# cita-cloud/consensus_overlord

Hardware: AMD Instinct MI355X
Metric: BLS12-381 vote verifications/sec (batch 4096) at 1/2/4/8 MI355X vs host blst (higher is better)
Workload: dtype u32; 1 GPU; config3: 4096 distinct-message precommit votes per GPU, RLC batch verify; batch_per_gpu=4096, global_batch=4096, parallelism=single GPU

## Files before the change

### consensus_overlord_amd/csrc/fpvm.hpp

```cpp
#pragma once
#include "bls/fp.hpp"

#if defined(__HIPCC__)
#define VM_FN __device__ __forceinline__
#else
#define VM_FN inline
struct uint4 {
  uint32_t x, y, z, w;
};
inline uint4 make_uint4(uint32_t a, uint32_t b, uint32_t c, uint32_t d) { return uint4{a, b, c, d}; }
#endif

namespace ovh {
namespace vm {

enum : uint32_t {
  OP_NOP = 0, OP_MULS = 1, OP_SGN0 = 2, OP_LEX = 3, OP_INV = 4, OP_LIN = 5, OP_SEL = 6, OP_EQ = 7,
  OP_AND = 8, OP_OR = 9, OP_XOR = 10, OP_ST = 11, OP_SELB = 12,
};

constexpr uint32_t PREFETCH = 6;

struct Out {
  uint32_t* base;
  uint32_t cap;
  uint32_t unit;
};
constexpr uint32_t CONST_BASE = 0x800;
constexpr uint32_t KZERO = 1, KTAB = 2;

VM_FN void ld_slot(Fp& r, const uint32_t* __restrict__ slots, const uint32_t* __restrict__ cst,
                   uint32_t ref) {
  const uint32_t* src = ((ref & CONST_BASE) ? cst : slots) + (ref & (CONST_BASE - 1)) * 12;
  const uint4* s4 = reinterpret_cast<const uint4*>(src);
  const uint4 a = s4[0], b = s4[1], c = s4[2];
  r.v[0] = a.x; r.v[1] = a.y; r.v[2] = a.z; r.v[3] = a.w;
  r.v[4] = b.x; r.v[5] = b.y; r.v[6] = b.z; r.v[7] = b.w;
  r.v[8] = c.x; r.v[9] = c.y; r.v[10] = c.z; r.v[11] = c.w;
}

VM_FN const uint4* slot_ptr(const uint32_t* __restrict__ slots, const uint32_t* __restrict__ cst, uint32_t ref) {
  return reinterpret_cast<const uint4*>(((ref & CONST_BASE) ? cst : slots) + (ref & (CONST_BASE - 1)) * 12);
}

#if defined(__HIPCC__)
typedef uint32_t u32x4 __attribute__((ext_vector_type(4)));
typedef const __attribute__((address_space(3))) uint32_t* lds_cptr;
VM_FN uint32_t lds_addr(const uint32_t* __restrict__ slots, const uint32_t* __restrict__ cst, uint32_t ref) {
  return (uint32_t)(uintptr_t)(lds_cptr)(((ref & CONST_BASE) ? cst : slots) + (ref & (CONST_BASE - 1)) * 12);
}
VM_FN void unpack4(Fp& r, int q, const u32x4 v) {
  r.v[4 * q] = v.x; r.v[4 * q + 1] = v.y; r.v[4 * q + 2] = v.z; r.v[4 * q + 3] = v.w;
}
#endif

VM_FN void ld_slots4(Fp& A, Fp& B, Fp& C, Fp& D, const uint32_t* __restrict__ slots,
                     const uint32_t* __restrict__ cst, uint32_t ra, uint32_t rb, uint32_t rc, uint32_t rd) {
#if defined(__HIPCC__) && defined(OVH_VM_ASM_LOADS)
  const uint32_t xa = lds_addr(slots, cst, ra), xb = lds_addr(slots, cst, rb), xc = lds_addr(slots, cst, rc),
                 xd = lds_addr(slots, cst, rd);
  u32x4 b0, d0, a0, c0, b1, d1, a1, c1, b2, d2, a2, c2;
  asm volatile(
      "ds_read_b128 %0, %12\n\tds_read_b128 %1, %13\n\tds_read_b128 %2, %14\n\tds_read_b128 %3, %15\n\t"
      "ds_read_b128 %4, %12 offset:16\n\tds_read_b128 %5, %13 offset:16\n\t"
      "ds_read_b128 %6, %14 offset:16\n\tds_read_b128 %7, %15 offset:16\n\t"
      "ds_read_b128 %8, %12 offset:32\n\tds_read_b128 %9, %13 offset:32\n\t"
      "ds_read_b128 %10, %14 offset:32\n\tds_read_b128 %11, %15 offset:32"
      : "=&v"(b0), "=&v"(d0), "=&v"(a0), "=&v"(c0), "=&v"(b1), "=&v"(d1), "=&v"(a1), "=&v"(c1), "=&v"(b2),
        "=&v"(d2), "=&v"(a2), "=&v"(c2)
      : "v"(xb), "v"(xd), "v"(xa), "v"(xc)
      : "memory");
  asm volatile("s_waitcnt lgkmcnt(8)" : "+v"(b0), "+v"(d0), "+v"(a0), "+v"(c0));
  unpack4(B, 0, b0); unpack4(D, 0, d0); unpack4(A, 0, a0); unpack4(C, 0, c0);
  asm volatile("s_waitcnt lgkmcnt(4)" : "+v"(b1), "+v"(d1), "+v"(a1), "+v"(c1));
  unpack4(B, 1, b1); unpack4(D, 1, d1); unpack4(A, 1, a1); unpack4(C, 1, c1);
  asm volatile("s_waitcnt lgkmcnt(0)" : "+v"(b2), "+v"(d2), "+v"(a2), "+v"(c2));
  unpack4(B, 2, b2); unpack4(D, 2, d2); unpack4(A, 2, a2); unpack4(C, 2, c2);
  return;
#endif
#if defined(__HIP_DEVICE_COMPILE__)
  typedef const __attribute__((address_space(3))) u32x4* lds_q;
  const uint32_t sb = (uint32_t)(uintptr_t)(lds_cptr)slots, cb = (uint32_t)(uintptr_t)(lds_cptr)cst;
  auto addr = [&](uint32_t ref) -> lds_q {
    const uint32_t m = (uint32_t)__builtin_amdgcn_sbfe((int32_t)ref, 11, 1);
    uint32_t base;
    asm("v_bfi_b32 %0, %1, %2, %3" : "=v"(base) : "v"(m), "v"(cb), "v"(sb));
    return (lds_q)(uintptr_t)(__builtin_amdgcn_ubfe(ref, 0, 11) * 48u + base);
  };
  const lds_q pa = addr(ra), pb = addr(rb), pc = addr(rc), pd = addr(rd);
#else
  const uint4 *pa = slot_ptr(slots, cst, ra), *pb = slot_ptr(slots, cst, rb), *pc = slot_ptr(slots, cst, rc),
              *pd = slot_ptr(slots, cst, rd);
#endif
#pragma unroll
  for (int q = 0; q < 3; ++q) {
#if defined(__HIP_DEVICE_COMPILE__)
    const u32x4 b = pb[q], d = pd[q], a = pa[q], c = pc[q];
#else
    const uint4 b = pb[q], d = pd[q], a = pa[q], c = pc[q];
#endif
    B.v[4 * q] = b.x; B.v[4 * q + 1] = b.y; B.v[4 * q + 2] = b.z; B.v[4 * q + 3] = b.w;
    D.v[4 * q] = d.x; D.v[4 * q + 1] = d.y; D.v[4 * q + 2] = d.z; D.v[4 * q + 3] = d.w;
    A.v[4 * q] = a.x; A.v[4 * q + 1] = a.y; A.v[4 * q + 2] = a.z; A.v[4 * q + 3] = a.w;
    C.v[4 * q] = c.x; C.v[4 * q + 1] = c.y; C.v[4 * q + 2] = c.z; C.v[4 * q + 3] = c.w;
#if defined(__HIPCC__)
    __builtin_amdgcn_sched_barrier(0);
#endif
  }
}

VM_FN void st_slot(uint32_t* __restrict__ slots, uint32_t dst, const Fp& z) {
  uint4* d4 = reinterpret_cast<uint4*>(slots + dst * 12);
  d4[0] = make_uint4(z.v[0], z.v[1], z.v[2], z.v[3]);
  d4[1] = make_uint4(z.v[4], z.v[5], z.v[6], z.v[7]);
  d4[2] = make_uint4(z.v[8], z.v[9], z.v[10], z.v[11]);
}

VM_FN void set_flag(Fp& z, uint32_t f) {
  fp_zero(z);
  z.v[0] = f;
}

constexpr uint32_t P2_LIMBS[12] = {
    P_LIMBS[0] << 1, (P_LIMBS[1] << 1) | (P_LIMBS[0] >> 31), (P_LIMBS[2] << 1) | (P_LIMBS[1] >> 31),
    (P_LIMBS[3] << 1) | (P_LIMBS[2] >> 31), (P_LIMBS[4] << 1) | (P_LIMBS[3] >> 31),
    (P_LIMBS[5] << 1) | (P_LIMBS[4] >> 31), (P_LIMBS[6] << 1) | (P_LIMBS[5] >> 31),
    (P_LIMBS[7] << 1) | (P_LIMBS[6] >> 31), (P_LIMBS[8] << 1) | (P_LIMBS[7] >> 31),
    (P_LIMBS[9] << 1) | (P_LIMBS[8] >> 31), (P_LIMBS[10] << 1) | (P_LIMBS[9] >> 31),
    (P_LIMBS[11] << 1) | (P_LIMBS[10] >> 31)};

VM_FN void canon(Fp& r, const Fp& a) {
  uint32_t d[12], br = 0;
#pragma unroll
  for (int j = 0; j < 12; ++j) d[j] = subc32(a.v[j], P_LIMBS[j], br, &br);
#pragma unroll
  for (int j = 0; j < 12; ++j) r.v[j] = br ? a.v[j] : d[j];
}

constexpr uint32_t NP_LIMBS[12] = {
    0u - P_LIMBS[0], ~P_LIMBS[1], ~P_LIMBS[2], ~P_LIMBS[3], ~P_LIMBS[4], ~P_LIMBS[5],
    ~P_LIMBS[6], ~P_LIMBS[7], ~P_LIMBS[8], ~P_LIMBS[9], ~P_LIMBS[10], ~P_LIMBS[11]};
static_assert(P_LIMBS[0] != 0, "NP_LIMBS: no borrow out of limb 0");

VM_FN uint32_t quot_est(uint32_t t) {
  constexpr float QS = (float)((1.0 - 0x1p-20) / (double)((P_LIMBS[11] >> 7) + 1));
  return (uint32_t)((float)t * QS);
}

VM_FN void scale_reduce(Fp& r, const uint32_t* s, uint32_t k) {
  const uint32_t q = quot_est(k * (uint32_t)((((uint64_t)s[12] << 32) | s[11]) >> 7));
  uint64_t acc = 0;
#pragma unroll
  for (int j = 0; j < 12; ++j) {
    acc = (uint64_t)k * s[j] + (acc >> 32);
    acc = (uint64_t)q * NP_LIMBS[j] + acc;
    r.v[j] = (uint32_t)acc;
  }
}

constexpr uint32_t P2P1_LIMBS[12] = {
    P2_LIMBS[0] + 1, P2_LIMBS[1], P2_LIMBS[2], P2_LIMBS[3], P2_LIMBS[4], P2_LIMBS[5],
    P2_LIMBS[6], P2_LIMBS[7], P2_LIMBS[8], P2_LIMBS[9], P2_LIMBS[10], P2_LIMBS[11]};

VM_FN void lin_mad(Fp& r, const Fp& A, const Fp& B, const Fp& C, const Fp& D, int ca, int cb, int cc, int cd) {
  const Fp* X[4] = {&A, &B, &C, &D};
  const int cf[4] = {ca, cb, cc, cd};
  uint64_t acc[12];
#pragma unroll
  for (int j = 0; j < 12; ++j) acc[j] = 0;
  uint32_t nw = 0;
#pragma unroll
  for (int t = 0; t < 4; ++t) {
    const uint32_t a = cf[t] < 0 ? (uint32_t)(-cf[t]) : (uint32_t)cf[t];
    const uint32_t m = cf[t] < 0 ? ~0u : 0u;
    nw += a & m;
#pragma unroll
    for (int j = 0; j < 12; ++j) acc[j] = (uint64_t)a * (X[t]->v[j] ^ m) + acc[j];
  }
#pragma unroll
  for (int j = 0; j < 12; ++j) acc[j] = (uint64_t)nw * P2P1_LIMBS[j] + acc[j];
  const int64_t top = (int64_t)(acc[11] >> 7) - ((int64_t)nw << 25);
  const uint32_t q = top > 0 ? quot_est((uint32_t)top) : 0u;
  uint64_t cy = 0;
#pragma unroll
  for (int j = 0; j < 12; ++j) {
    const uint64_t v = (uint64_t)q * NP_LIMBS[j] + (acc[j] + cy);
    r.v[j] = (uint32_t)v;
    cy = v >> 32;
  }
}

VM_FN void pre_add2(Fp& x, const Fp& A, const Fp& B, Fp& y, const Fp& C, const Fp& D, bool ny, bool any_neg) {
  uint32_t c1 = 0, c2 = 0;
  if (any_neg) {
    uint32_t nd[12], b2 = 0;
#pragma unroll
    for (int j = 0; j < 13; ++j) {
      if (j < 12) {
        nd[j] = subc32(P2_LIMBS[j], D.v[j], b2, &b2);
        x.v[j] = addc32(A.v[j], B.v[j], c1, &c1);
      }
      if (j >= 1) y.v[j - 1] = addc32(C.v[j - 1], ny ? nd[j - 1] : D.v[j - 1], c2, &c2);
    }
  } else {
#pragma unroll
    for (int j = 0; j < 12; ++j) {
      x.v[j] = addc32(A.v[j], B.v[j], c1, &c1);
      y.v[j] = addc32(C.v[j], D.v[j], c2, &c2);
    }
  }
}

constexpr uint32_t H_MUL = 1u << 22, H_MULNEG = 1u << 23, H_FLAG = 1u << 24, H_LIN = 1u << 25,
                   H_LINNEG = 1u << 26, H_ACC = 1u << 27, H_RARE = 1u << 28, H_SELB = 1u << 29,
                   H_LINNEG2 = 1u << 30, H_LINNEG3 = 1u << 31;
constexpr uint32_t H_ANY = H_MUL | H_LIN | H_ACC | H_RARE;

template <bool XB, bool XC>
VM_FN void lin_chain_neg(uint32_t* s, const Fp& A, const Fp& B, const Fp& C, const Fp& D, uint32_t mb, uint32_t mc,
                         uint32_t md, const Fp& K) {
  uint32_t u[12], v[12], w[12], c1 = 0, c2 = 0, c3 = 0, c4 = 0;
#pragma unroll
  for (int j = 0; j < 14; ++j) {
    if (j < 12) {
      u[j] = addc32(A.v[j], XB ? B.v[j] ^ mb : B.v[j], c1, &c1);
      v[j] = addc32(XC ? C.v[j] ^ mc : C.v[j], D.v[j] ^ md, c2, &c2);
    }
    if (j >= 1 && j <= 12) w[j - 1] = addc32(u[j - 1], v[j - 1], c3, &c3);
    if (j >= 2) s[j - 2] = addc32(w[j - 2], K.v[j - 2], c4, &c4);
  }
}

VM_FN void lin_sum(uint32_t* s, const Fp& A, const Fp& B, const Fp& C, const Fp& D, uint32_t mb, uint32_t mc,
                   uint32_t md, uint32_t hdr, const uint32_t* __restrict__ cst) {
  if (hdr & H_LINNEG) {
    const uint32_t n = (mb & 1u) + (mc & 1u) + (md & 1u);
    Fp K;
    ld_slot(K, nullptr, cst, CONST_BASE + KTAB + n);
    if (hdr & H_LINNEG3) {
      lin_chain_neg<true, true>(s, A, B, C, D, mb, mc, md, K);
    } else if (hdr & H_LINNEG2) {
#if defined(__HIP_DEVICE_COMPILE__)
      __asm__ volatile("");
#endif
      lin_chain_neg<false, true>(s, A, B, C, D, mb, mc, md, K);
    } else {
#if defined(__HIP_DEVICE_COMPILE__)
      __asm__ volatile("");
#endif
      lin_chain_neg<false, false>(s, A, B, C, D, mb, mc, md, K);
    }
  } else {
    uint32_t u[12], v[12], c1 = 0, c2 = 0, c3 = 0;
#pragma unroll
    for (int j = 0; j < 13; ++j) {
      if (j < 12) {
        u[j] = addc32(A.v[j], B.v[j], c1, &c1);
        v[j] = addc32(C.v[j], D.v[j], c2, &c2);
      }
      if (j >= 1) s[j - 1] = addc32(u[j - 1], v[j - 1], c3, &c3);
    }
  }
  s[12] = 0;
}

VM_FN void fp_inv(Fp& r, const Fp& a, const Fp& r3) { fp_inv_divsteps(r, a, r3); }

#if defined(__HIPCC__)
VM_FN uint32_t uniform(uint32_t w0) { return __builtin_amdgcn_readfirstlane(w0); }
#else
inline uint32_t uniform(uint32_t w0) { return w0; }
#endif

VM_FN uint32_t sign_mask(uint32_t w, int bit) { return (uint32_t)((int32_t)(w << (31 - bit)) >> 31); }
VM_FN int coef5(uint32_t w, int lo) { return ((int)(w << (27 - lo))) >> 27; }

VM_FN void exec(const uint4 in, bool active, uint32_t* __restrict__ slots, const uint32_t* __restrict__ cst,
                uint64_t scalar, const Out& out) {
  const uint32_t hdr = uniform(in.x);
  if (!(hdr & H_ANY)) return;
  const uint32_t op = active ? (in.x & 31) : (uint32_t)OP_NOP;
  uint32_t ra = in.y & 0xFFFF, rb = in.y >> 16, rc = in.z & 0xFFFF;
  bool selb = false;
  if (hdr & H_SELB) {
#if defined(__HIP_DEVICE_COMPILE__)
    __asm__ volatile("");
#endif
    selb = op == OP_SELB;
    const bool bit = ((scalar >> ((in.x >> 16) & 63)) & 1) != 0;
    ra = selb ? (bit ? rc : rb) : ra;
    rb = selb ? CONST_BASE + KZERO : rb;
    rc = selb ? CONST_BASE + KZERO : rc;
  }
  Fp A, B, C, D;
  ld_slots4(A, B, C, D, slots, cst, ra, rb, rc, in.z >> 16);
  const uint32_t dst = (in.x >> 5) & 0x7FF;
  const bool force_acc = (in.w & (1u << 24)) != 0;
  if (hdr & H_MUL) {
    const bool is_mul = op == OP_MULS || op == OP_SGN0 || op == OP_LEX || op == OP_EQ;
    Fp x, y, m;
    pre_add2(x, A, B, y, C, D, sign_mask(in.w, 19) != 0, (hdr & H_MULNEG) != 0);
    fp_mul(m, x, y);
    if (hdr & H_FLAG) {
      const bool flag = is_mul && op != OP_MULS;
      uint32_t f = 0;
      if (op == OP_SGN0) f = m.v[0] & 1u;
      if (op == OP_LEX) f = limbs_gt(m.v, HALF_P) ? 1u : 0u;
      if (op == OP_EQ) f = fp_is_zero(m) ? 1u : 0u;
#pragma unroll
      for (int j = 0; j < 12; ++j) m.v[j] = flag ? (j == 0 ? f : 0u) : m.v[j];
    }
    if (is_mul) st_slot(slots, dst, m);
  }
  if (hdr & H_LIN) {
    uint32_t s[13];
    lin_sum(s, A, B, C, D, sign_mask(in.w, 9), sign_mask(in.w, 14), sign_mask(in.w, 19), hdr, cst);
    const uint32_t k = (in.w >> 20) & 15;
    Fp l;
    scale_reduce(l, s, k > 1 ? k : 1u);
    if ((op == OP_LIN && !force_acc) || selb) st_slot(slots, dst, l);
  }
  if (hdr & H_ACC) {
    Fp l;
    lin_mad(l, A, B, C, D, coef5(in.w, 0), coef5(in.w, 5), coef5(in.w, 10), coef5(in.w, 15));
    if (op == OP_LIN && force_acc) st_slot(slots, dst, l);
  }
  if (hdr & H_RARE) {
    const bool rare = op != OP_NOP && op != OP_LIN && !selb && op != OP_MULS && op != OP_SGN0 && op != OP_LEX &&
                      op != OP_EQ;
    const uint32_t imm = (in.x >> 16) & 63;
    Fp z = A;
    if (op == OP_ST) {
      canon(z, A);
      uint32_t* b = out.base + (size_t)imm * 12 * out.cap + out.unit;
#pragma unroll
      for (int k = 0; k < 12; ++k) b[(size_t)k * out.cap] = z.v[k];
    } else if (op == OP_SEL) {
      z = A.v[0] ? C : B;
    } else if (op >= OP_AND && op <= OP_XOR) {
      set_flag(z, op == OP_AND ? (A.v[0] & C.v[0]) : op == OP_OR ? (A.v[0] | C.v[0]) : (A.v[0] ^ C.v[0]));
    } else if (op == OP_INV) {
#ifndef OVH_VM_NO_INV
      Fp a;
      canon(a, A);
      fp_inv(z, a, C);
#endif
    }
    if (rare && op != OP_ST) st_slot(slots, dst, z);
  }
#if defined(__HIP_DEVICE_COMPILE__)
  __asm__ volatile("" ::"v"(A.v[11]), "v"(B.v[11]), "v"(C.v[11]), "v"(D.v[11]));
#endif
}

#if defined(__HIPCC__)
constexpr uint32_t SIDE_VALID = 1u << 31, SIDE_FILL = 1u << 30;

__device__ __forceinline__ void side_spill(uint32_t sw, uint32_t* __restrict__ slots, uint32_t* __restrict__ scr) {
  if ((sw & (SIDE_VALID | SIDE_FILL)) == SIDE_VALID) {
    const u32x4* s = reinterpret_cast<const u32x4*>(slots + (sw & 0x7FF) * 12);
    const u32x4 a = s[0], b = s[1], c = s[2];
    u32x4* d = reinterpret_cast<u32x4*>(scr + ((sw >> 11) & 0xFFF) * 12);
    d[0] = a;
    d[1] = b;
    d[2] = c;
  }
}

template <bool SIDE = false>
__device__ __forceinline__ void run(const uint4* __restrict__ code, uint32_t nphases, uint32_t W, uint32_t lane,
                                    bool active, uint32_t* __restrict__ slots, const uint32_t* __restrict__ cst,
                                    uint64_t scalar, const Out& out, uint64_t* __restrict__ trace = nullptr,
                                    const uint32_t* __restrict__ side = nullptr, uint32_t* __restrict__ scr = nullptr) {
  static_assert(PREFETCH >= 5, "the unrolled loops below read up to 4 phases past the end");
  if constexpr (SIDE) {
    uint4 qa = code[lane], qb = code[W + lane], qc;
    uint32_t sa = side[lane], sb = side[W + lane], sc;
    if (!active) sa = sb = 0;
    __builtin_amdgcn_s_waitcnt(0x0F70);
    auto step = [&](const uint4& q, uint4& q2, const uint32_t s, const uint32_t sn, uint32_t& s2,
                    const uint32_t ph) __attribute__((always_inline)) {
      const bool fill = (sn & (SIDE_VALID | SIDE_FILL)) == (SIDE_VALID | SIDE_FILL);
      u32x4 f0, f1, f2;
      if (fill) {
        const u32x4* src = reinterpret_cast<const u32x4*>(scr + ((sn >> 11) & 0xFFF) * 12);
        f0 = __builtin_nontemporal_load(src);
        f1 = __builtin_nontemporal_load(src + 1);
        f2 = __builtin_nontemporal_load(src + 2);
      }
      q2 = code[(size_t)(ph + 2) * W + lane];
      s2 = active ? side[(size_t)(ph + 2) * W + lane] : 0u;
      exec(q, active, slots, cst, scalar, out);
      side_spill(s, slots, scr);
      if (fill) {
        u32x4* d = reinterpret_cast<u32x4*>(slots + (sn & 0x7FF) * 12);
        d[0] = f0;
        d[1] = f1;
        d[2] = f2;
      }
    };
#pragma unroll 1
    for (uint32_t ph = 0; ph < nphases; ph += 3) {
      step(qa, qc, sa, sb, sc, ph);
      step(qb, qa, sb, sc, sa, ph + 1);
      step(qc, qb, sc, sa, sb, ph + 2);
    }
    __asm__ volatile("s_waitcnt lgkmcnt(0)\n\ts_barrier" ::: "memory");
    return;
  }
  if (trace && threadIdx.x == 0) trace[0] = wall_clock64();
  uint4 qa = code[lane], qb = code[W + lane], qc;
  __builtin_amdgcn_s_waitcnt(0x0F70);
  auto step = [&](const uint4& q, uint4& q2, const uint32_t ph) __attribute__((always_inline)) {
    q2 = code[(size_t)(ph + 2) * W + lane];
    exec(q, active, slots, cst, scalar, out);
    if (trace && ph < nphases) {
      __asm__ volatile("s_waitcnt lgkmcnt(0)" ::: "memory");
      if (threadIdx.x == 0) trace[ph + 1] = wall_clock64();
    }
  };
#pragma unroll 1
  for (uint32_t ph = 0; ph < nphases; ph += 3) {
    step(qa, qc, ph);
    step(qb, qa, ph + 1);
    step(qc, qb, ph + 2);
  }
  __asm__ volatile("s_waitcnt lgkmcnt(0)\n\ts_barrier" ::: "memory");
}

#endif

}
}
```

### consensus_overlord_amd/csrc/msm.hpp

```cpp
#pragma once

#define MSM_NBW 255
#define MSM_NB (4 * MSM_NBW)
#define MSM_NT 32
#define MSM_TM 64
#define MSM_LV 27
#define MSM_U (MSM_NT * MSM_TM)
#define MSM_CH_LV 6
#define MSM_CH (1u << MSM_CH_LV)
#define MSM_PF_ROWS 2

struct MsmArgs {
  const uint32_t* cnt;
  const uint32_t* off;
  const uint32_t* pf;
  const uint32_t* ent;
  Slab st;
  Slab A;
  Slab U;
};

__device__ __forceinline__ uint32_t msm_half(uint64_t r, uint32_t h) { return h ? (uint32_t)(r >> 32) : (uint32_t)r; }

#define MSM_TPB 64

__global__ __launch_bounds__(MSM_TPB) void k_msm_zero(uint32_t* __restrict__ cnt) {
  const uint32_t k = blockIdx.x * MSM_TPB + threadIdx.x;
  if (k < MSM_NB) cnt[k] = 0;
}

__global__ __launch_bounds__(MSM_TPB) void k_msm_count(uint32_t n, uint64_t seed, uint64_t base,
                                                       const int32_t* __restrict__ codes, uint32_t* __restrict__ cnt) {
  __shared__ uint32_t h[MSM_NB];
  for (uint32_t k = threadIdx.x; k < MSM_NB; k += MSM_TPB) h[k] = 0;
  __syncthreads();
  const uint32_t i = blockIdx.x * MSM_TPB + threadIdx.x;
  if (i < n && codes[i] == 0) {
    const uint64_t r = vote_scalar(seed, base, i);
    for (uint32_t hh = 0; hh < 2; ++hh) {
      const uint32_t s = msm_half(r, hh);
      for (uint32_t w = 0; w < 4; ++w) {
        const uint32_t d = (s >> (8 * w)) & 255u;
        if (d) atomicAdd(&h[w * MSM_NBW + d - 1], 1u);
      }
    }
  }
  __syncthreads();
  for (uint32_t k = threadIdx.x; k < MSM_NB; k += MSM_TPB)
    if (h[k]) atomicAdd(&cnt[k], h[k]);
}

template <class F, class G>
__device__ __forceinline__ uint32_t wave_scan_nb(F v, G out) {
  static_assert(MSM_NB <= 16 * 64, "16 entries per lane");
  const uint32_t t = threadIdx.x;
  uint32_t loc[16], sum = 0;
#pragma unroll
  for (int j = 0; j < 16; ++j) {
    const uint32_t b = 16 * t + j;
    loc[j] = b < MSM_NB ? v(b) : 0u;
    sum += loc[j];
  }
  uint32_t incl = sum;
#pragma unroll
  for (int d = 1; d < 64; d <<= 1) {
    const uint32_t x = __shfl_up(incl, d, 64);
    if (t >= (uint32_t)d) incl += x;
  }
  uint32_t run = incl - sum;
#pragma unroll
  for (int j = 0; j < 16; ++j) {
    const uint32_t b = 16 * t + j;
    if (b < MSM_NB) out(b, run);
    run += loc[j];
  }
  return __shfl(incl, 63, 64);
}

__global__ __launch_bounds__(64) void k_msm_scan(const uint32_t* __restrict__ cnt, uint32_t* __restrict__ off,
                                                 uint32_t* __restrict__ cur, uint32_t* __restrict__ pf) {
  const uint32_t tot = wave_scan_nb([&](uint32_t b) { return cnt[b]; },
                                    [&](uint32_t b, uint32_t e) {
                                      off[b] = e;
                                      cur[b] = e;
                                    });
  if (threadIdx.x == 0) off[MSM_NB] = tot;
  for (uint32_t row = 0; row < MSM_PF_ROWS; ++row) {
    uint32_t* p = pf + (size_t)row * (MSM_NB + 1);
    const uint32_t t = wave_scan_nb(
        [&](uint32_t b) {
          const uint32_t c = cnt[b];
          return row == 0 ? (c + 1) / 2 : (c + MSM_CH - 1) >> MSM_CH_LV;
        },
        [&](uint32_t b, uint32_t e) { p[b] = e; });
    if (threadIdx.x == 0) p[MSM_NB] = t;
  }
}

__global__ __launch_bounds__(MSM_TPB) void k_msm_scatter(uint32_t n, uint64_t seed, uint64_t base,
                                                         const int32_t* __restrict__ codes, uint32_t* __restrict__ cur,
                                                         uint32_t* __restrict__ ent) {
  const uint32_t i = blockIdx.x * MSM_TPB + threadIdx.x;
  if (i >= n || codes[i] != 0) return;
  const uint64_t r = vote_scalar(seed, base, i);
  for (uint32_t hh = 0; hh < 2; ++hh) {
    const uint32_t s = msm_half(r, hh);
    for (uint32_t w = 0; w < 4; ++w) {
      const uint32_t d = (s >> (8 * w)) & 255u;
      if (d) ent[atomicAdd(&cur[w * MSM_NBW + d - 1], 1u)] = 2 * i + hh;
    }
  }
}

__global__ __launch_bounds__(64) void k_sig_as_S(Slab st, const int32_t* __restrict__ codes, Slab U) {
  const uint32_t c = threadIdx.x;
  if (c >= 6) return;
  Fp v;
  const bool ok = codes[0] == 0;
  if (ok && c < 4) st.ld(v, S_SIG + c, 0);
  else if (c == (ok ? 4u : 2u)) fp_one(v);
  else fp_zero(v);
  U.st(v, c, 0);
}

enum : uint32_t { SRC_ID = 0, SRC_PT = 1, SRC_A = 2, SRC_U = 3 };

__device__ __forceinline__ uint32_t msm_find(const uint32_t* __restrict__ row, uint32_t q) {
  uint32_t lo = 0, hi = MSM_NB;
  while (hi - lo > 1) {
    const uint32_t mid = (lo + hi) >> 1;
    if (row[mid] <= q) lo = mid;
    else hi = mid;
  }
  return lo;
}

__device__ __forceinline__ uint32_t msm_member(uint32_t j, uint32_t k) {
  return ((j >> k) << (k + 1)) | (1u << k) | (j & ((1u << k) - 1));
}

__device__ __forceinline__ void msm_coord(Fp& v, const MsmArgs& a, uint32_t kind, uint32_t idx, uint32_t c) {
  if (kind == SRC_PT) {
    if (c < 4) a.st.ld(v, ((idx & 1) ? S_TAU : S_SIG) + c, idx >> 1);
    else if (c == 4) fp_one(v);
    else fp_zero(v);
  } else if (kind == SRC_A) {
    a.A.ld(v, c, idx);
  } else if (kind == SRC_U) {
    a.U.ld(v, c, idx);
  } else if (c == 2) {
    fp_one(v);
  } else {
    fp_zero(v);
  }
}

template <int W>
__device__ __forceinline__ void msm_pair_op(const VmDev& prog, uint32_t nin, uint32_t* slots, const uint32_t* cst,
                                            uint32_t lane, bool active, const MsmArgs& a, uint32_t ka, uint32_t ia,
                                            uint32_t kb, uint32_t ib, uint32_t kd, uint32_t id) {
  if (active) {
    const uint32_t na = nin - 6;
    for (uint32_t k = lane; k < nin; k += W) {
      Fp v;
      if (k < na) msm_coord(v, a, ka, ia, k);
      else msm_coord(v, a, kb, ib, k - na);
      slot_put(slots, prog.in[k], v.v);
    }
  }
  __syncthreads();
  vm::run(prog.code, prog.nphases, W, lane, active, slots, cst, 0, vm::Out{nullptr, 0, 0});
  if (active) {
    const Slab& d = kd == SRC_U ? a.U : a.A;
    for (uint32_t k = lane; k < 6; k += W) {
      Fp v;
      const uint32_t src = prog.out[k];
      for (int l = 0; l < 12; ++l) v.v[l] = slots[src * 12 + l];
      vm::canon(v, v);
      d.st(v, k, id);
    }
  }
  __syncthreads();
}

__device__ __forceinline__ VmDev msm_prog(bool first, const VmDev& x, const VmDev& y) {
  VmDev r;
  r.code = first ? x.code : y.code;
  r.nphases = first ? x.nphases : y.nphases;
  r.in = first ? x.in : y.in;
  r.out = first ? x.out : y.out;
  r.trace = nullptr, r.clk = nullptr, r.side = nullptr;
  return r;
}

#define MSM_VM_PROLOGUE(W)                                    \
  __builtin_amdgcn_s_setprio(3);                              \
  extern __shared__ uint4 lds4[];                             \
  uint32_t* lds = reinterpret_cast<uint32_t*>(lds4);          \
  const uint32_t* cst = lds;                                  \
  const uint32_t slice = threadIdx.x / (W), lane = threadIdx.x % (W); \
  uint32_t* slots = lds + SLOT_BASE_W + slice * stride_w;     \
  load_consts(lds, cst_g, VM_NCONST)

__global__ __launch_bounds__(64) void k_msm_chunk(VmDev madd, VmDev padd, uint32_t stride_w,
                                                  const uint32_t* __restrict__ cst_g, MsmArgs a) {
  constexpr uint32_t W = VM_MADD_W, SL = 64 / W;
  const uint32_t* rowc = a.pf + (MSM_NB + 1);
  if (blockIdx.x >= rowc[MSM_NB]) return;
  MSM_VM_PROLOGUE(W);
  const uint32_t b = msm_find(rowc, blockIdx.x), k0 = (blockIdx.x - rowc[b]) << MSM_CH_LV;
  const uint32_t c = a.cnt[b], a0 = a.pf[b], e0 = a.off[b];
  const uint32_t m = c - k0 < MSM_CH ? c - k0 : MSM_CH;
  for (uint32_t lv = 0; lv < MSM_CH_LV && (lv == 0 || (1u << lv) < m); ++lv) {
    const uint32_t h = 1u << lv;
    const uint32_t np = lv == 0 ? (m + 1) / 2 : (m - h + 2 * h - 1) >> (lv + 1);
    const VmDev prog = msm_prog(lv == 0, madd, padd);
    for (uint32_t r = 0; r < np; r += SL) {
      const uint32_t p = r + slice, k = k0 + (p << (lv + 1));
      const bool act = p < np;
      uint32_t ka = SRC_A, ia = a0 + (k >> 1), kb = SRC_A, ib = a0 + ((k + h) >> 1);
      const uint32_t id = ia;
      if (lv == 0) {
        ka = SRC_PT, kb = SRC_ID, ia = ib = 0;
        if (act) {
          ia = a.ent[e0 + k];
          if (k + 1 < c) kb = SRC_PT, ib = a.ent[e0 + k + 1];
        }
      }
      msm_pair_op<W>(prog, lv == 0 ? VM_MADD_NIN : VM_PADD_NIN, slots, cst, lane, act, a, ka, ia, kb, ib, SRC_A, id);
    }
  }
}

__global__ __launch_bounds__(64) void k_msm_upper(VmDev padd, uint32_t stride_w, const uint32_t* __restrict__ cst_g,
                                                  MsmArgs a) {
  constexpr uint32_t W = VM_PADD_W, SL = 64 / W;
  const uint32_t c = a.cnt[blockIdx.x];
  if (c <= MSM_CH) return;
  MSM_VM_PROLOGUE(W);
  const uint32_t a0 = a.pf[blockIdx.x];
  for (uint32_t lv = MSM_CH_LV; (1u << lv) < c; ++lv) {
    const uint32_t h = 1u << lv, np = (c - h + 2 * h - 1) >> (lv + 1);
    for (uint32_t r = 0; r < np; r += SL) {
      const uint32_t p = r + slice, k = p << (lv + 1);
      const uint32_t ia = a0 + (k >> 1), ib = a0 + ((k + h) >> 1);
      msm_pair_op<W>(padd, VM_PADD_NIN, slots, cst, lane, p < np, a, SRC_A, ia, SRC_A, ib, SRC_A, ia);
    }
  }
}

__global__ __launch_bounds__(64) void k_msm_plane(uint32_t lo, uint32_t hi, VmDev padd, uint32_t stride_w,
                                                  const uint32_t* __restrict__ cst_g, MsmArgs a) {
  constexpr uint32_t W = VM_PADD_W, SL = 64 / W;
  MSM_VM_PROLOGUE(W);
  const uint32_t per_t = MSM_TM >> hi, t = blockIdx.x / per_t, g = blockIdx.x % per_t;
  for (uint32_t lv = lo; lv <= hi; ++lv) {
    const uint32_t np = 1u << (hi - lv);
    for (uint32_t r = 0; r < np; r += SL) {
      const uint32_t p = r + slice, i = g * np + p;
      const bool act = p < np;
      uint32_t ka = SRC_U, ia = t * MSM_TM + (i << lv), kb = SRC_U, ib = ia + (lv ? 1u << (lv - 1) : 0u);
      const uint32_t id = ia;
      if (lv == 0) {
        ka = kb = SRC_ID, ia = ib = 0;
        if (act) {
          const uint32_t w = t >> 3, k = t & 7;
          const uint32_t b0 = w * MSM_NBW + msm_member(2 * i, k) - 1, b1 = w * MSM_NBW + msm_member(2 * i + 1, k) - 1;
          if (a.cnt[b0]) ka = SRC_A, ia = a.pf[b0];
          if (a.cnt[b1]) kb = SRC_A, ib = a.pf[b1];
        }
      }
      msm_pair_op<W>(padd, VM_PADD_NIN, slots, cst, lane, act, a, ka, ia, kb, ib, SRC_U, id);
    }
  }
}

__global__ __launch_bounds__(64) void k_msm_comb(uint32_t lo, uint32_t hi, VmDev p0, VmDev p1, VmDev p2,
                                                 uint32_t stride_w, const uint32_t* __restrict__ cst_g, MsmArgs a) {
  constexpr uint32_t W = VM_HDBL1_W, SL = 64 / W;
  MSM_VM_PROLOGUE(W);
  for (uint32_t h = lo; h <= hi; ++h) {
    const VmDev prog = msm_prog(h == lo, p0, msm_prog(h == lo + 1, p1, p2));
    const uint32_t np = 1u << (hi - h), m = 1u << (h - 1);
    for (uint32_t r = 0; r < np; r += SL) {
      const uint32_t p = r + slice, e = 2 * m * (blockIdx.x * np + p) * MSM_TM;
      msm_pair_op<W>(prog, VM_HDBL1_NIN, slots, cst, lane, p < np, a, SRC_U, e, SRC_U, e + m * MSM_TM, SRC_U, e);
    }
  }
}
```

### consensus_overlord_amd/csrc/ovhip.hip

```cpp
#include <hip/hip_runtime.h>

#include <errno.h>
#include <stdlib.h>
#include <sys/random.h>
#include <sys/types.h>

#include <algorithm>
#include <atomic>
#include <deque>
#include <mutex>
#include <new>
#include <string>
#include <string.h>
#include <unordered_map>
#include <vector>

#include "../../include/ovhip.h"
#include "bls/verify.hpp"
#include "fpvm.hpp"
#include "keygen.hpp"
#include "rlp.hpp"
#include "sm3.hpp"
#ifdef OVH_VM_PROGS
#include OVH_VM_PROGS
#else
#include <vm_progs.inc>
#endif
static_assert(VM_KZERO == ovh::vm::KZERO && VM_KTAB == ovh::vm::KTAB, "fixed constants (tools/fpvm/gen.py)");

using namespace ovh;

#define WG 64

struct Slab {
  uint32_t* p;
  uint32_t cap;
  __device__ __forceinline__ void ld(Fp& a, uint32_t j, uint32_t i) const {
    const uint32_t* b = p + (size_t)j * 12 * cap + i;
#pragma unroll
    for (int k = 0; k < 12; ++k) a.v[k] = b[(size_t)k * cap];
  }
  __device__ __forceinline__ void st(const Fp& a, uint32_t j, uint32_t i) const {
    uint32_t* b = p + (size_t)j * 12 * cap + i;
#pragma unroll
    for (int k = 0; k < 12; ++k) b[(size_t)k * cap] = a.v[k];
  }
  __device__ void ld2(Fp2& a, uint32_t j, uint32_t i) const {
    ld(a.c0, j, i);
    ld(a.c1, j + 1, i);
  }
  __device__ void st2(const Fp2& a, uint32_t j, uint32_t i) const {
    st(a.c0, j, i);
    st(a.c1, j + 1, i);
  }
  __device__ void ld_g2j(G2J& a, uint32_t i) const {
    ld2(a.X, 0, i);
    ld2(a.Y, 2, i);
    ld2(a.Z, 4, i);
  }
  __device__ void st_g2j(const G2J& a, uint32_t i) const {
    st2(a.X, 0, i);
    st2(a.Y, 2, i);
    st2(a.Z, 4, i);
  }
  __device__ void ld_g2a(G2A& a, uint32_t i) const {
    ld2(a.x, 0, i);
    ld2(a.y, 2, i);
  }
  __device__ void st_g2a(const G2A& a, uint32_t i) const {
    st2(a.x, 0, i);
    st2(a.y, 2, i);
  }
  __device__ void ld_g1a(G1A& a, uint32_t i) const {
    ld(a.x, 0, i);
    ld(a.y, 1, i);
  }
  __device__ void st_g1a(const G1A& a, uint32_t i) const {
    st(a.x, 0, i);
    st(a.y, 1, i);
  }
  __device__ void ld_f12(Fp12& f, uint32_t i) const {
    Fp* c = &f.c0.c0.c0;
    for (int j = 0; j < 12; ++j) ld(c[j], j, i);
  }
  __device__ void st_f12(const Fp12& f, uint32_t i) const {
    const Fp* c = &f.c0.c0.c0;
    for (int j = 0; j < 12; ++j) st(c[j], j, i);
  }
};

enum : uint32_t {
  S_U = VM_S_U,
  S_SIG = VM_S_SIG,
  S_TAU = VM_S_TAU,
  S_F = VM_S_F,
  S_RS = VM_S_RS,
  S_TOTAL = VM_S_TOTAL,
};
constexpr uint32_t PART_PLANES = 18;
constexpr size_t FIN_STRIDE = (size_t)PART_PLANES * 12 * 20;

enum : int { ST_H2F = 0, ST_VOTE, ST_FOLD, ST_FINAL, ST_FALLBACK, ST_MSM };
static_assert(ST_MSM + 1 == OVH_NSTAGES, "stage table");

__device__ __forceinline__ uint64_t rlc_scalar(uint64_t seed, uint64_t i) {
  uint64_t z = seed + 0x9e3779b97f4a7c15ull * (i + 1);
  z = (z ^ (z >> 30)) * 0xbf58476d1ce4e5b9ull;
  z = (z ^ (z >> 27)) * 0x94d049bb133111ebull;
  z = z ^ (z >> 31);
  return z ? z : 1;
}

#define UNIT_BASE 0xFFFFFFFFFFFFFFFFull
__device__ __forceinline__ uint64_t vote_scalar(uint64_t seed, uint64_t base, uint64_t i) {
  return base == UNIT_BASE ? 1ull : rlc_scalar(seed, base + i);
}

__global__ __launch_bounds__(WG) void k_vote_digest(uint32_t n, const uint64_t* __restrict__ heights,
                                                    const uint64_t* __restrict__ rounds,
                                                    const uint8_t* __restrict__ types, const uint8_t* __restrict__ bh,
                                                    const uint8_t* __restrict__ lens, uint8_t* __restrict__ out) {
  const uint32_t i = blockIdx.x * WG + threadIdx.x;
  if (i >= n) return;
  uint8_t h[VOTE_HASH_MAX];
  const uint32_t len = lens[i];
  uint8_t d[32];
  if (len > VOTE_HASH_MAX) {
    for (int k = 0; k < 32; ++k) out[(size_t)i * 32 + k] = 0;
    return;
  }
  for (uint32_t k = 0; k < len; ++k) h[k] = bh[(size_t)i * VOTE_HASH_MAX + k];
  vote_digest(d, heights[i], rounds[i], types[i], h, len);
  for (int k = 0; k < 32; ++k) out[(size_t)i * 32 + k] = d[k];
}

__global__ __launch_bounds__(WG) void k_h2f(uint32_t n, const uint8_t* __restrict__ hashes, XmdTemplates t, Slab s) {
  const uint32_t i = blockIdx.x * WG + threadIdx.x;
  if (i >= n) return;
  uint32_t msg[8], uni[64];
  be_words_from_bytes(msg, hashes + (size_t)i * 32, 8);
  expand_message_xmd_256(uni, msg, t);
  Fp2 u0, u1;
  hash_to_field_fp2x2(u0, u1, uni);
  s.st2(u0, S_U, i);
  s.st2(u1, S_U + 2, i);
}

__device__ void parse_hdr(const uint8_t* b, uint32_t nbytes, uint32_t* x_hi, uint32_t* x_lo, uint32_t& bad,
                          uint32_t& inf, uint32_t& sort, uint32_t& xzero) {
  const uint8_t b0 = b[0];
  bad = 0;
  inf = 0;
  sort = (b0 >> 5) & 1u;
  xzero = 0;
  uint8_t t[48];
  for (int i = 0; i < 48; ++i) t[i] = b[i];
  t[0] &= 0x1f;
  limbs_from_be48(x_hi, t);
  if (nbytes == 96) limbs_from_be48(x_lo, b + 48);
  if (!(b0 & 0x80)) {
    bad = 1;
    return;
  }
  if (b0 & 0x40) {
    uint32_t acc = b0 & 0x3f;
    for (uint32_t i = 1; i < nbytes; ++i) acc |= b[i];
    if (acc) bad = 1;
    else inf = 1;
    return;
  }
  if (!limbs_lt_p(x_hi)) bad = 1;
  if (nbytes == 96 && !limbs_lt_p(x_lo)) bad = 1;
  uint32_t z = 0;
  for (int k = 0; k < 12; ++k) z |= x_hi[k] | (nbytes == 96 ? x_lo[k] : 0u);
  xzero = z == 0;
}

struct VmDev {
  const uint4* code;
  uint32_t nphases;
  const uint16_t* in;
  const uint16_t* out;
  uint64_t* trace;
  uint64_t* clk;
  const uint32_t* side;
};
constexpr uint32_t VOTE_NSCR = VM_VOTE_NSCR > VM_VOTE_T_NSCR ? VM_VOTE_NSCR : VM_VOTE_T_NSCR;

#define VM_CLOCK_WGS (1u << 16)
struct ClockStamp {
  uint64_t t0 = 0, r0 = 0;
  __device__ __forceinline__ void begin(const uint64_t* clk) {
    if (clk && threadIdx.x == 0) {
      t0 = __builtin_amdgcn_s_memtime();
      r0 = __builtin_amdgcn_s_memrealtime();
    }
  }
  __device__ __forceinline__ void end(uint64_t* clk) {
    if (clk && threadIdx.x == 0 && blockIdx.x < VM_CLOCK_WGS) {
      const uint64_t t1 = __builtin_amdgcn_s_memtime(), r1 = __builtin_amdgcn_s_memrealtime();
      clk[2 * blockIdx.x] = t1 - t0;
      clk[2 * blockIdx.x + 1] = r1 - r0;
    }
  }
};

#ifndef SMALL_MAX
#define SMALL_MAX 1024u
#endif
#define VM_SLICES 4
constexpr uint32_t align128w(uint32_t w) { return (w + 31) / 32 * 32; }
constexpr uint32_t align256w(uint32_t w) { return (w + 63) / 64 * 64; }
constexpr uint32_t SLOT_BASE_W = align256w(VM_NCONST * 12);
constexpr uint32_t VOTE_STRIDE_W = align256w(VM_VOTE_NSLOTS * 12 + 4);
constexpr uint32_t VOTE_T_STRIDE_W = align256w(VM_VOTE_T_NSLOTS * 12 + 4);
constexpr uint32_t FOLD_STRIDE_W = align128w(VM_FOLD_NSLOTS * 12);
#define VM_FOLD_UNITS (64 / VM_FOLD_W)

__device__ __forceinline__ void load_consts(uint32_t* cst, const uint32_t* __restrict__ g, uint32_t n) {
  for (uint32_t k = threadIdx.x; k < n * 12; k += blockDim.x) cst[k] = g[k];
}

__device__ __forceinline__ void slot_flag(uint32_t* slots, uint32_t s, uint32_t f) {
  uint4* d = reinterpret_cast<uint4*>(slots + s * 12);
  d[0] = make_uint4(f, 0, 0, 0);
  d[1] = make_uint4(0, 0, 0, 0);
  d[2] = make_uint4(0, 0, 0, 0);
}

__device__ __forceinline__ void slot_put(uint32_t* slots, uint32_t s, const uint32_t* v) {
  for (int k = 0; k < 12; ++k) slots[s * 12 + k] = v[k];
}

__device__ __forceinline__ uint32_t slot_flag_get(const uint32_t* slots, uint32_t s) { return slots[s * 12]; }

__device__ __forceinline__ void fold_unit(uint32_t t, uint32_t m, const VmDev& prog, const uint32_t* cst,
                                          uint32_t* slots, uint32_t lane, bool active, Slab inF, Slab inS,
                                          Slab out, const int32_t* __restrict__ codes) {
  if (active) {
    for (uint32_t k = lane; k < 4 * PART_PLANES; k += VM_FOLD_W) {
      const uint32_t q = k / PART_PLANES, j = k % PART_PLANES, e = 4 * t + q;
      Fp v;
      if (e < m && (!codes || codes[e] == 0) && (j < 12 || inS.p)) {
        if (j < 12) inF.ld(v, j, e);
        else inS.ld(v, j - 12, e);
      } else if (j == 0 || j == 12 + 2) {
        fp_one(v);
      } else {
        fp_zero(v);
      }
      slot_put(slots, VM_FOLD_IN[k], v.v);
    }
  }
  __syncthreads();
  vm::run(prog.code, VM_FOLD_NPHASES, VM_FOLD_W, lane, active, slots, cst, 0, vm::Out{nullptr, 0, 0});
  if (active) {
    for (uint32_t k = lane; k < PART_PLANES; k += VM_FOLD_W) {
      Fp v;
      const uint32_t src = VM_FOLD_OUT[k];
      for (int q = 0; q < 12; ++q) v.v[q] = slots[src * 12 + q];
      vm::canon(v, v);
      out.st(v, k, t);
    }
  }
}

#ifndef OVH_VOTE_STAGGER
#define OVH_VOTE_STAGGER 12
#endif
__device__ __forceinline__ void vote_stagger() {
#if OVH_VOTE_STAGGER > 0
  const uint32_t hw = __builtin_amdgcn_s_getreg((31 << 11) | 4);
  const uint32_t n = ((hw >> 4) & 3) * OVH_VOTE_STAGGER;
#pragma unroll 1
  for (uint32_t k = 0; k < n; ++k) __builtin_amdgcn_s_sleep(1);
#endif
}

#define PKF_PARSE 1u
#define PKF_INF 2u
#define PKF_GRP 4u
struct PkSrc {
  const uint32_t* planes;
  uint32_t cap;
  const uint32_t* flags;
  const int32_t* idx;
};

#define POOL_SEQR 16u
#define POOL_QW 16u
enum : uint32_t {
  PQ_CUR = 0,
  PQ_NPUB = POOL_QW,
  PQ_SLOTOF = 2 * POOL_QW,
  PQ_NANN = 3 * POOL_QW,
  PQ_DONE = 4 * POOL_QW,
  PQ_CLAIM = PQ_DONE + OVH_BATCH_SLOTS * POOL_QW,
  PQ_INFL = PQ_CLAIM + OVH_BATCH_SLOTS * POOL_QW,
  PQ_OCC = PQ_INFL + POOL_QW,
};
constexpr uint32_t POOL_OCC_N = 4096;
constexpr uint32_t PQ_WORDS = PQ_OCC + POOL_OCC_N / 2;
static_assert(POOL_SEQR > OVH_BATCH_SLOTS && POOL_SEQR / 2 <= POOL_QW, "pool queue layout");
#define POOL_IDLE_TICKS 2000ull
#define POOL_WAIT_TICKS 2000000ull

__device__ __forceinline__ uint32_t simd_key() {
  const uint32_t hw = __builtin_amdgcn_s_getreg((31 << 11) | 4);
  const uint32_t xcc = __builtin_amdgcn_s_getreg((3 << 11) | 20);
  return (xcc & 7u) << 9 | ((hw >> 13) & 3u) << 7 | ((hw >> 12) & 1u) << 6 | ((hw >> 8) & 15u) << 2 |
         ((hw >> 4) & 3u);
}
__device__ __forceinline__ uint32_t* pq_occ(uint64_t* q) { return reinterpret_cast<uint32_t*>(q + PQ_OCC); }
#define POOL_SPREAD_TICKS 20000ull

struct PoolBatch {
  uint64_t seq;
  uint32_t n, nq;
  uint32_t table;
  uint32_t has_idx;
  uint64_t seed, base;
  int32_t* codes;
  const uint32_t* planes;
  const uint32_t* flags;
  uint32_t pcap, cap;
  uint32_t* state;
  uint32_t* part0;
  const uint8_t* stage;
  uint64_t* clk;
  uint32_t part_cap, pad;
  uint64_t* plog;
};

#define PLOG_RING 64u
#define PLOG_QUADS 1024u
#define PLOG_WORDS (16u + 2u * PLOG_QUADS)
#define PLOG_GRIDS 64u
#define PLOG_WGS 1024u
#define PLOG_WG_WORDS 4u
#define PLOG_GRID_BASE ((size_t)PLOG_RING * PLOG_WORDS)
#define PLOG_TOTAL (PLOG_GRID_BASE + (size_t)PLOG_GRIDS * (4 + PLOG_WGS * PLOG_WG_WORDS))
enum : uint32_t { PLOG_EV_PUB = 0, PLOG_EV_DONE = 1, PLOG_EV_FOLD = 2, PLOG_EV_MSM = 3, PLOG_EV_FINAL = 4,
                  PLOG_EV_BACK = 5, PLOG_EV_GATH = 6, PLOG_EV_COMB = 7, PLOG_EV_FE = 8, PLOG_EV_SEQ = 15 };
__global__ void k_grid_hdr(uint64_t* g, uint64_t seq, uint32_t par, uint32_t wgs) {
  for (uint32_t k = threadIdx.x; k < PLOG_WGS * PLOG_WG_WORDS; k += blockDim.x) g[4 + k] = 0;
  __syncthreads();
  if (threadIdx.x == 0) {
    g[0] = seq;
    g[1] = par;
    g[2] = wgs;
    g[3] = __builtin_amdgcn_s_memrealtime();
  }
}
__global__ void k_stamp(uint64_t* p, uint64_t v) {
  if (threadIdx.x == 0) {
    p[0] = __builtin_amdgcn_s_memrealtime();
    if (v != ~0ull) p[PLOG_EV_SEQ] = v;
  }
}

struct PoolArgs {
  uint64_t* q;
  const PoolBatch* descs;
  const uint4* pv_code;
  const uint32_t* pv_side;
  const uint4* pt_code;
  const uint32_t* pt_side;
  const uint4* fold_code;
  const uint32_t* cst;
  uint32_t* scr;
  uint64_t* wlog;
  uint64_t only;
  uint32_t nsimd;
  uint32_t skip_cu;
};

__device__ __forceinline__ uint64_t* pq_done(uint64_t* q, uint32_t slot) { return q + PQ_DONE + slot * POOL_QW; }
__device__ __forceinline__ uint64_t* pq_claim(uint64_t* q, uint32_t slot) { return q + PQ_CLAIM + slot * POOL_QW; }
__device__ __forceinline__ uint32_t* pq_slot_of(uint64_t* q) { return reinterpret_cast<uint32_t*>(q + PQ_SLOTOF); }
__device__ __forceinline__ uint64_t qld(const uint64_t* p) {
  return __hip_atomic_load(p, __ATOMIC_RELAXED, __HIP_MEMORY_SCOPE_AGENT);
}

__global__ __launch_bounds__(64) void k_pool_publish(PoolBatch b, uint32_t slot, uint64_t seq, uint64_t* q,
                                                     PoolBatch* descs) {
  if (threadIdx.x) return;
  b.seq = ~0ull;
  descs[slot] = b;
  __builtin_amdgcn_fence(__ATOMIC_RELEASE, "agent");
  asm volatile("s_waitcnt vmcnt(0)" ::: "memory");
  __hip_atomic_store(&descs[slot].seq, seq, __ATOMIC_RELAXED, __HIP_MEMORY_SCOPE_AGENT);
  __hip_atomic_store(pq_done(q, slot), 0ull, __ATOMIC_RELAXED, __HIP_MEMORY_SCOPE_AGENT);
  __hip_atomic_store(pq_claim(q, slot), seq << 32, __ATOMIC_RELAXED, __HIP_MEMORY_SCOPE_AGENT);
  __hip_atomic_store(pq_slot_of(q) + seq % POOL_SEQR, slot, __ATOMIC_RELAXED, __HIP_MEMORY_SCOPE_AGENT);
  __builtin_amdgcn_fence(__ATOMIC_RELEASE, "agent");
  asm volatile("s_waitcnt vmcnt(0)" ::: "memory");
  __hip_atomic_store(q + PQ_NPUB, seq + 1, __ATOMIC_RELAXED, __HIP_MEMORY_SCOPE_AGENT);
}

__global__ __launch_bounds__(64) void k_pool_announce(uint64_t* q, uint64_t n) {
  if (threadIdx.x == 0) __hip_atomic_store(q + PQ_NANN, n, __ATOMIC_RELAXED, __HIP_MEMORY_SCOPE_AGENT);
}

__device__ __forceinline__ uint64_t lane0_fetch_add(uint64_t* p, uint64_t v) {
  uint64_t r = 0;
  if (threadIdx.x == 0) r = __hip_atomic_fetch_add(p, v, __ATOMIC_RELAXED, __HIP_MEMORY_SCOPE_AGENT);
  return ((uint64_t)__builtin_amdgcn_readfirstlane((uint32_t)(r >> 32)) << 32) |
         __builtin_amdgcn_readfirstlane((uint32_t)r);
}
__device__ __forceinline__ uint32_t lane0_fetch_add32(uint32_t* p, uint32_t v) {
  uint32_t r = 0;
  if (threadIdx.x == 0) r = __hip_atomic_fetch_add(p, v, __ATOMIC_RELAXED, __HIP_MEMORY_SCOPE_AGENT);
  return __builtin_amdgcn_readfirstlane(r);
}
__device__ __forceinline__ void lane0_cas(uint64_t* p, uint64_t expect, uint64_t want) {
  if (threadIdx.x == 0) {
    uint64_t e = expect;
    (void)__hip_atomic_compare_exchange_strong(p, &e, want, __ATOMIC_RELAXED, __ATOMIC_RELAXED,
                                               __HIP_MEMORY_SCOPE_AGENT);
  }
}
__device__ __forceinline__ uint64_t wclock() {
  const uint64_t t = wall_clock64();
  return ((uint64_t)__builtin_amdgcn_readfirstlane((uint32_t)(t >> 32)) << 32) | __builtin_amdgcn_readfirstlane((uint32_t)t);
}
__device__ __forceinline__ uint64_t qldu(const uint64_t* p) {
  const uint64_t v = __hip_atomic_load(p, __ATOMIC_RELAXED, __HIP_MEMORY_SCOPE_AGENT);
  return ((uint64_t)__builtin_amdgcn_readfirstlane((uint32_t)(v >> 32)) << 32) | __builtin_amdgcn_readfirstlane((uint32_t)v);
}
__device__ uint32_t pool_claim(uint64_t* q, const PoolBatch* descs, uint32_t* slot_out, uint32_t* quad_out,
                               uint32_t* why, uint64_t only, uint32_t nsimd, uint32_t* how) {
  uint64_t t0 = wclock(), tdef = 0;
  uint32_t hw = 0;
  uint32_t* occ = pq_occ(q) + simd_key();
  *why = 3;
#pragma unroll 1
  for (uint32_t tries = 0; tries < (1u << 22); ++tries) {
    const uint64_t s = qldu(q + PQ_CUR), np = qldu(q + PQ_NPUB);
    if (s > only) {
      *why = 4;
      return 0;
    }
    if (s >= np) {
      const uint64_t idle = wclock() - t0;
      if (idle > POOL_WAIT_TICKS ||
          (idle > POOL_IDLE_TICKS && qldu(q + PQ_NANN) <= np && qldu(q + PQ_INFL) == 0)) {
        *why = idle > POOL_WAIT_TICKS ? 2 : 1;
        return 0;
      }
      if (idle > POOL_IDLE_TICKS) __builtin_amdgcn_s_sleep(127);
      else __builtin_amdgcn_s_sleep(8);
      continue;
    }
    const uint32_t slot = __builtin_amdgcn_readfirstlane(
        __hip_atomic_load(pq_slot_of(q) + s % POOL_SEQR, __ATOMIC_RELAXED, __HIP_MEMORY_SCOPE_AGENT));
    bool held = false;
    if (np == s + 1) {
      hw |= 1u;
      bool busy;
      if (tdef && __builtin_amdgcn_readfirstlane(__hip_atomic_load(occ, __ATOMIC_RELAXED, __HIP_MEMORY_SCOPE_AGENT))) {
        busy = true;
      } else {
        busy = lane0_fetch_add32(occ, 1u) != 0;
        held = true;
      }
      if (busy) {
        hw |= 2u;
        const uint64_t cw = qldu(pq_claim(q, slot));
        const uint32_t nq = __builtin_amdgcn_readfirstlane(
            __hip_atomic_load(&descs[slot].nq, __ATOMIC_RELAXED, __HIP_MEMORY_SCOPE_AGENT));
        const uint64_t infl = qldu(q + PQ_INFL);
        const uint32_t taken = (uint32_t)cw;
        if ((cw >> 32) == s && taken < nq && (uint64_t)(nq - taken) + infl <= nsimd + nsimd / 16) {
          const uint64_t now = wclock();
          if (!tdef) tdef = now;
          if (now - tdef < POOL_SPREAD_TICKS) {
            hw |= 4u;
            if (held) (void)lane0_fetch_add32(occ, ~0u);
            __builtin_amdgcn_s_sleep(32);
            continue;
          }
        }
        hw |= 8u;
      }
    }
    if (!held) (void)lane0_fetch_add32(occ, 1u);
    const uint64_t old = lane0_fetch_add(pq_claim(q, slot), 1ull);
    const uint64_t seq = old >> 32;
    const uint32_t idx = (uint32_t)old;
    const uint64_t tw = wclock();
    while (qldu(q + PQ_NPUB) <= seq && wclock() - tw < 100000000ull) __builtin_amdgcn_s_sleep(2);
    const uint32_t nq = __builtin_amdgcn_readfirstlane(
        __hip_atomic_load(&descs[slot].nq, __ATOMIC_RELAXED, __HIP_MEMORY_SCOPE_AGENT));
    asm volatile("s_waitcnt vmcnt(0)" ::: "memory");
    const uint64_t dseq = qldu(&descs[slot].seq);
    const bool mine = dseq == seq && idx < nq;
    if (seq != s || !mine) lane0_cas(q + PQ_CUR, s, s + 1);
    if (mine) {
      (void)lane0_fetch_add(q + PQ_INFL, 1ull);
      *slot_out = slot;
      *quad_out = idx;
      *how = hw;
      return 1;
    }
    (void)lane0_fetch_add32(occ, ~0u);
    tdef = 0;
    t0 = wclock();
  }
  return 0;
}

template <typename T>
__device__ __forceinline__ T dget(const T* p) {
  return __hip_atomic_load(p, __ATOMIC_RELAXED, __HIP_MEMORY_SCOPE_AGENT);
}
template <typename T>
__device__ __forceinline__ T* dgetp(T* const* p) {
  return reinterpret_cast<T*>(__hip_atomic_load(reinterpret_cast<const uint64_t*>(p), __ATOMIC_RELAXED,
                                                __HIP_MEMORY_SCOPE_AGENT));
}
__device__ __forceinline__ uint32_t uni(uint32_t v) { return __builtin_amdgcn_readfirstlane(v); }
__device__ __forceinline__ uint64_t uni64(uint64_t v) {
  return ((uint64_t)uni((uint32_t)(v >> 32)) << 32) | uni((uint32_t)v);
}
template <typename T>
__device__ __forceinline__ T* unip(T* p) {
  return reinterpret_cast<T*>(uni64(reinterpret_cast<uint64_t>(p)));
}

template <bool TABLE>
__device__ __forceinline__ void vote_quad(const PoolArgs& a, uint32_t slot_in, uint32_t quad_in, uint32_t* lds) {
  constexpr uint32_t NSLOTS = TABLE ? VM_VOTE_T_NSLOTS : VM_VOTE_NSLOTS;
  constexpr uint32_t STRIDE = TABLE ? VOTE_T_STRIDE_W : VOTE_STRIDE_W;
  constexpr uint32_t NPH = TABLE ? VM_VOTE_T_NPHASES : VM_VOTE_NPHASES;
  const uint16_t* IN = TABLE ? VM_VOTE_T_IN : VM_VOTE_IN;
  const uint16_t* OUT = TABLE ? VM_VOTE_T_OUT : VM_VOTE_OUT;
  uint32_t* cst = lds;
  const uint32_t slice = threadIdx.x / VM_VOTE_W, lane = threadIdx.x % VM_VOTE_W;
  uint32_t* slots = lds + SLOT_BASE_W + slice * STRIDE;
  uint32_t* hdr = slots + NSLOTS * 12;
  uint32_t* park = lds + SLOT_BASE_W + 2 * STRIDE + NSLOTS * 12 + 2;
  {
    const PoolBatch* bd = a.descs + slot_in;
    const uint32_t i = (quad_in & 0x0FFFFFFFu) * VM_SLICES + slice;
    const uint32_t n = uni(dget(&bd->n));
    const bool active = i < n;
    const uint8_t* sigs = unip(dgetp(&bd->stage));
    const Slab s{unip(dgetp(&bd->state)), uni(dget(&bd->cap))};
    if (active) {
      if (lane == 0) {
        uint32_t x1[12], x0[12], bad, inf, sort, xz;
        parse_hdr(sigs + (size_t)i * 96, 96, x1, x0, bad, inf, sort, xz);
        slot_put(slots, IN[TABLE ? VM_VOTE_T_IN_SIG_X1 : VM_VOTE_IN_SIG_X1], x1);
        slot_put(slots, IN[TABLE ? VM_VOTE_T_IN_SIG_X0 : VM_VOTE_IN_SIG_X0], x0);
        slot_flag(slots, IN[TABLE ? VM_VOTE_T_IN_SIG_SORT : VM_VOTE_IN_SIG_SORT], sort);
        hdr[0] = bad | inf << 1 | xz << 2;
      } else if (lane >= 2 && lane < 6) {
        Fp u;
        s.ld(u, S_U + (lane - 2), i);
        slot_put(slots, IN[(TABLE ? VM_VOTE_T_IN_U00 : VM_VOTE_IN_U00) + (lane - 2)], u.v);
      }
    }
    if (threadIdx.x == 0) {
      park[0] = slot_in;
      park[1] = quad_in;
      if (dgetp(&bd->plog)) {
        uint32_t* h3 = lds + SLOT_BASE_W + 3 * STRIDE + NSLOTS * 12 + 2;
        const uint64_t t = __builtin_amdgcn_s_memrealtime();
        h3[0] = (uint32_t)t;
        h3[1] = (uint32_t)(t >> 32);
      }
    }
    __syncthreads();
    if (active) {
      if constexpr (TABLE) {
        const int32_t* idx = reinterpret_cast<const int32_t*>(sigs + (size_t)n * 144);
        const uint32_t e = uni(dget(&bd->has_idx)) ? (uint32_t)idx[i] : i;
        if (lane == 1) {
          hdr[1] = unip(dgetp(&bd->flags))[e];
        } else if (lane >= 6 && lane < 9) {
          Fp v;
          Slab{const_cast<uint32_t*>(unip(dgetp(&bd->planes))), uni(dget(&bd->pcap))}.ld(v, lane - 6, e);
          slot_put(slots, IN[VM_VOTE_T_IN_PK_X + (lane - 6)], v.v);
        }
      } else {
        if (lane == 1) {
          uint32_t x[12], bad, inf, sort, xz;
          parse_hdr(sigs + (size_t)n * 96 + (size_t)i * 48, 48, x, x, bad, inf, sort, xz);
          slot_put(slots, IN[VM_VOTE_IN_PK_X], x);
          slot_flag(slots, IN[VM_VOTE_IN_PK_SORT], sort);
          hdr[1] = bad | inf << 1 | xz << 2;
        }
      }
    }
    if (threadIdx.x == 0 && dgetp(&bd->clk)) {
      const uint64_t t0 = __builtin_amdgcn_s_memtime(), r0 = __builtin_amdgcn_s_memrealtime();
      uint32_t* h0 = lds + SLOT_BASE_W + NSLOTS * 12 + 2;
      uint32_t* h1 = lds + SLOT_BASE_W + STRIDE + NSLOTS * 12 + 2;
      h0[0] = (uint32_t)t0;
      h0[1] = (uint32_t)(t0 >> 32);
      h1[0] = (uint32_t)r0;
      h1[1] = (uint32_t)(r0 >> 32);
    }
    __syncthreads();
    const uint64_t scalar = vote_scalar(uni64(dget(&bd->seed)), uni64(dget(&bd->base)), i);
    vm::run<true>(TABLE ? a.pt_code : a.pv_code, NPH, VM_VOTE_W, lane, active, slots, cst, scalar,
                  vm::Out{s.p, s.cap, i}, nullptr, TABLE ? a.pt_side : a.pv_side,
                  a.scr + (size_t)blockIdx.x * VM_SLICES * VOTE_NSCR * 12 + slice * VOTE_NSCR * 12);
  }
  const uint32_t slot = uni(park[0]), quad = uni(park[1]) & 0x0FFFFFFFu, how = uni(park[1]) >> 28;
  const PoolBatch* bd = a.descs + slot;
  const uint32_t i = quad * VM_SLICES + slice;
  const uint32_t n = uni(dget(&bd->n));
  int32_t* codes = unip(dgetp(&bd->codes));
  if (uint64_t* clk = dgetp(&bd->clk); clk && threadIdx.x == 0 && blockIdx.x < VM_CLOCK_WGS) {
    const uint32_t* h0 = lds + SLOT_BASE_W + NSLOTS * 12 + 2;
    const uint32_t* h1 = lds + SLOT_BASE_W + STRIDE + NSLOTS * 12 + 2;
    const uint64_t t0 = h0[0] | (uint64_t)h0[1] << 32, r0 = h1[0] | (uint64_t)h1[1] << 32;
    clk[2 * blockIdx.x] = __builtin_amdgcn_s_memtime() - t0;
    clk[2 * blockIdx.x + 1] = __builtin_amdgcn_s_memrealtime() - r0;
  }
  if (i < n && lane == 0) {
    const uint32_t sf = hdr[0], pf = hdr[1];
    const uint32_t sg_bad = sf & 1, sg_inf = (sf >> 1) & 1, sg_xz = (sf >> 2) & 1;
    const uint32_t sg_ok = slot_flag_get(slots, OUT[TABLE ? VM_VOTE_T_OUT_SIG_OK : VM_VOTE_OUT_SIG_OK]);
    const uint32_t sg_grp = slot_flag_get(slots, OUT[TABLE ? VM_VOTE_T_OUT_SIG_GRP : VM_VOTE_OUT_SIG_GRP]);
    const uint32_t h_inf = slot_flag_get(slots, OUT[TABLE ? VM_VOTE_T_OUT_H_INF : VM_VOTE_OUT_H_INF]);
    uint32_t pk_parse, pk_inf, pk_grp;
    if constexpr (TABLE) {
      pk_parse = pf & PKF_PARSE;
      pk_inf = pf & PKF_INF;
      pk_grp = !(pf & PKF_GRP);
    } else {
      const uint32_t pk_bad = pf & 1, pk_xz = (pf >> 2) & 1;
      pk_inf = (pf >> 1) & 1;
      const uint32_t pk_ok = slot_flag_get(slots, OUT[VM_VOTE_OUT_PK_OK]);
      pk_grp = slot_flag_get(slots, OUT[VM_VOTE_OUT_PK_GRP]);
      pk_parse = pk_bad || (!pk_inf && (!pk_ok || pk_xz));
    }
    int32_t c;
    if (pk_parse) c = OVH_ERR_PUBKEY;
    else if (sg_bad) c = BLST_BAD_ENCODING;
    else if (!sg_inf && !sg_ok) c = BLST_POINT_NOT_ON_CURVE;
    else if (!sg_inf && (sg_xz || !sg_grp)) c = BLST_POINT_NOT_IN_GROUP;
    else if (pk_inf) c = BLST_PK_IS_INFINITY;
    else if (!pk_grp) c = BLST_POINT_NOT_IN_GROUP;
    else if (h_inf || sg_inf) c = BLST_VERIFY_FAIL;
    else c = 0;
    codes[i] = c;
  }
  __threadfence();
  __syncthreads();
  uint64_t* const pl = threadIdx.x == 0 && quad < PLOG_QUADS ? dgetp(&bd->plog) : nullptr;
  uint64_t pl_start = 0;
  if (pl) {
    const uint32_t* h3 = lds + SLOT_BASE_W + 3 * STRIDE + NSLOTS * 12 + 2;
    pl_start = (uint64_t)h3[0] | (uint64_t)(h3[1] & 0xFFFFu) << 32;
  }
  const Slab s{unip(dgetp(&bd->state)), uni(dget(&bd->cap))};
  VmDev fold{};
  fold.code = a.fold_code;
  fold_unit(quad, n, fold, cst, lds + SLOT_BASE_W, threadIdx.x % VM_FOLD_W, threadIdx.x < VM_FOLD_W,
            Slab{s.p + (size_t)S_F * 12 * s.cap, s.cap}, Slab{nullptr, 0},
            Slab{unip(dgetp(&bd->part0)), uni(dget(&bd->part_cap))}, codes);
  if (pl) {
    pl[16 + 2 * quad] = pl_start | (uint64_t)simd_key() << 48 | (uint64_t)how << 60;
    pl[16 + 2 * quad + 1] = __builtin_amdgcn_s_memrealtime();
  }
  __builtin_amdgcn_fence(__ATOMIC_RELEASE, "agent");
  asm volatile("s_waitcnt vmcnt(0)" ::: "memory");
  if (threadIdx.x == 0) {
    __hip_atomic_fetch_add(pq_done(a.q, slot), 1ull, __ATOMIC_RELAXED, __HIP_MEMORY_SCOPE_AGENT);
    __hip_atomic_fetch_add(a.q + PQ_INFL, ~0ull, __ATOMIC_RELAXED, __HIP_MEMORY_SCOPE_AGENT);
    __hip_atomic_fetch_add(pq_occ(a.q) + simd_key(), ~0u, __ATOMIC_RELAXED, __HIP_MEMORY_SCOPE_AGENT);
  }
}

__global__ __launch_bounds__(64, 2) void k_vm_pool(PoolArgs a) {
  __builtin_amdgcn_s_setprio(2);
  extern __shared__ uint4 lds4[];
  if (a.skip_cu && ((simd_key() >> 2) & 0x7Fu) < a.skip_cu) return;
  uint32_t* lds = reinterpret_cast<uint32_t*>(lds4);
  load_consts(lds, a.cst, VM_NCONST);
  const uint64_t t_in = __builtin_amdgcn_s_memrealtime();
  vote_stagger();
  uint32_t nquads = 0, why = 0;
#pragma unroll 1
  for (;; ++nquads) {
    uint32_t slot = 0, quad = 0, how = 0;
    if (!pool_claim(a.q, a.descs, &slot, &quad, &why, a.only, a.nsimd, &how)) break;
    slot = uni(slot);
    quad = uni(quad) | uni(how) << 28;
    __builtin_amdgcn_fence(__ATOMIC_ACQUIRE, "agent");
    if (uni(dget(&a.descs[slot].table))) vote_quad<true>(a, slot, quad, lds);
    else vote_quad<false>(a, slot, quad, lds);
  }
  if (a.wlog && threadIdx.x == 0 && blockIdx.x < PLOG_WGS) {
    uint64_t* w = a.wlog + (size_t)blockIdx.x * PLOG_WG_WORDS;
    w[0] = t_in;
    w[1] = __builtin_amdgcn_s_memrealtime();
    w[2] = nquads;
    w[3] = why;
  }
}

__global__ __launch_bounds__(64) void k_pool_wait(uint64_t* q, uint32_t slot, uint32_t nq, uint64_t ticks,
                                                  uint32_t* err) {
  if (threadIdx.x) return;
  const uint64_t t0 = wall_clock64();
  while (__hip_atomic_load(pq_done(q, slot), __ATOMIC_RELAXED, __HIP_MEMORY_SCOPE_AGENT) < nq) {
    if (wall_clock64() - t0 > ticks) {
      __hip_atomic_store(err, 1u, __ATOMIC_RELAXED, __HIP_MEMORY_SCOPE_SYSTEM);
      return;
    }
    __builtin_amdgcn_s_sleep(32);
  }
}

__global__ __launch_bounds__(WG) void k_pool_stage(uint32_t n, const uint8_t* __restrict__ sigs,
                                                   const uint8_t* __restrict__ pks, const int32_t* __restrict__ idx,
                                                   uint8_t* __restrict__ dst) {
  const size_t nb = (size_t)n * 96 + (pks ? (size_t)n * 48 : 0);
  uint8_t* di = dst + (size_t)n * 144;
  for (size_t k = (size_t)blockIdx.x * WG + threadIdx.x; k < nb + (idx ? (size_t)n * 4 : 0);
       k += (size_t)gridDim.x * WG) {
    if (k < (size_t)n * 96) dst[k] = sigs[k];
    else if (k < nb) dst[k] = pks[k - (size_t)n * 96];
    else di[k - nb] = reinterpret_cast<const uint8_t*>(idx)[k - nb];
  }
}

template <int SLICES>
__global__ __launch_bounds__(64) void k_vm_fold(uint32_t m, VmDev prog, const uint32_t* __restrict__ cst_g, Slab inF,
                                                Slab inS, Slab out, const int32_t* __restrict__ codes,
                                                const int32_t* __restrict__ gate = nullptr) {
  if (gate && *gate == 1) return;
  __builtin_amdgcn_s_setprio(2);
  extern __shared__ uint4 lds4[];
  uint32_t* lds = reinterpret_cast<uint32_t*>(lds4);
  uint32_t* cst = lds;
  const uint32_t slice = threadIdx.x / VM_FOLD_W, lane = threadIdx.x % VM_FOLD_W;
  const uint32_t sl = slice < SLICES ? slice : 0;
  uint32_t* slots = lds + SLOT_BASE_W + sl * FOLD_STRIDE_W;
  const uint32_t t = blockIdx.x * SLICES + slice;
  const bool active = slice < SLICES && 4 * t < m;
  load_consts(cst, cst_g, VM_NCONST);
  fold_unit(t, m, prog, cst, slots, lane, active, inF, inS, out, codes);
}

__global__ __launch_bounds__(64) void k_vm_final(uint32_t m, VmDev prog, const uint32_t* __restrict__ cst_g, Slab inF,
                                                 Slab inS, Slab xS, int32_t* __restrict__ result) {
  __builtin_amdgcn_s_setprio(3);
  extern __shared__ uint4 lds4[];
  uint32_t* lds = reinterpret_cast<uint32_t*>(lds4);
  uint32_t* cst = lds;
  uint32_t* slots = lds + SLOT_BASE_W;
  const uint32_t lane = threadIdx.x;
  load_consts(cst, cst_g, VM_NCONST);
  for (uint32_t k = lane; k < 4 * PART_PLANES; k += 64) {
    const uint32_t q = k / PART_PLANES, j = k % PART_PLANES;
    Fp v;
    if (q == 0 && j >= 12 && xS.p) {
      xS.ld(v, j - 12, 0);
    } else if (q < m) {
      if (j < 12) inF.ld(v, j, q);
      else inS.ld(v, j - 12, q);
    } else if (j == 0 || j == 12 + 2) {
      fp_one(v);
    } else {
      fp_zero(v);
    }
    slot_put(slots, VM_FINAL_IN[k], v.v);
  }
  __syncthreads();
  vm::run(prog.code, VM_FINAL_NPHASES, VM_FINAL_W, lane, true, slots, cst, 0, vm::Out{nullptr, 0, 0},
          blockIdx.x == 0 ? prog.trace : nullptr);
  if (lane == 0) *result = slot_flag_get(slots, VM_FINAL_OUT[0]) ? 1 : 0;
}

static_assert(VM_VOTEW_NIN == VM_VOTE1_NIN && VM_VOTEW_T_NIN == VM_VOTE_T1_NIN && VM_VOTEW_W == 64 &&
                  VM_VOTEW_T_W == 64 && VM_VOTE1_W == 64 && VM_VOTE_T1_W == 64,
              "one-vote-per-wave programs share the vote1 / vote_t1 layouts");
static_assert(VM_VOTE1H_IN_H0 == VM_VOTE1_IN_U00 && VM_VOTE_T1H_IN_H0 == VM_VOTE_T1_IN_U00 &&
                  VM_VOTE1H_OUT_SIG_GRP == VM_VOTE1_OUT_SIG_GRP && VM_VOTE_T1H_OUT_SIG_GRP == VM_VOTE_T1_OUT_SIG_GRP,
              "vote1h / vote_t1h share vote1 / vote_t1's layouts, H in place of the u's");
template <bool TABLE, bool HIN = false>
__device__ __forceinline__ void vote_wave(const VmDev& prog, uint32_t nph, uint32_t ns, const uint16_t* IN,
                                          const uint16_t* OUT, const uint32_t* __restrict__ cst_g,
                                          const uint8_t* __restrict__ pk_bytes, PkSrc pk, uint32_t e,
                                          const uint8_t* __restrict__ sig, Slab s, uint32_t i, uint64_t scalar,
                                          int32_t* __restrict__ code, Slab hc = Slab{nullptr, 0}, uint32_t he = 0,
                                          const uint32_t* __restrict__ hinf_in = nullptr,
                                          uint32_t* __restrict__ hinf_out = nullptr) {
  extern __shared__ uint4 lds4[];
  uint32_t* lds = reinterpret_cast<uint32_t*>(lds4);
  uint32_t* cst = lds;
  uint32_t* slots = lds + SLOT_BASE_W;
  uint32_t* hdr = slots + ns * 12;
  const uint32_t lane = threadIdx.x;
  load_consts(cst, cst_g, VM_NCONST);
  if (lane == 0) {
    uint32_t x1[12], x0[12], bad, inf, sort, xz;
    parse_hdr(sig, 96, x1, x0, bad, inf, sort, xz);
    if constexpr (TABLE) {
      slot_put(slots, IN[VM_VOTE_T1_IN_SIG_X1], x1);
      slot_put(slots, IN[VM_VOTE_T1_IN_SIG_X0], x0);
      slot_flag(slots, IN[VM_VOTE_T1_IN_SIG_SORT], sort);
    } else {
      slot_put(slots, IN[VM_VOTE1_IN_SIG_X1], x1);
      slot_put(slots, IN[VM_VOTE1_IN_SIG_X0], x0);
      slot_flag(slots, IN[VM_VOTE1_IN_SIG_SORT], sort);
    }
    hdr[0] = bad | inf << 1 | xz << 2;
  } else if (lane == 1) {
    if constexpr (TABLE) {
      hdr[1] = pk.flags[e];
    } else {
      uint32_t x[12], bad, inf, sort, xz;
      parse_hdr(pk_bytes, 48, x, x, bad, inf, sort, xz);
      slot_put(slots, IN[VM_VOTE1_IN_PK_X], x);
      slot_flag(slots, IN[VM_VOTE1_IN_PK_SORT], sort);
      hdr[1] = bad | inf << 1 | xz << 2;
    }
  } else if (!HIN && lane >= 2 && lane < 6) {
    Fp u;
    s.ld(u, S_U + (lane - 2), i);
    if constexpr (TABLE) slot_put(slots, IN[VM_VOTE_T1_IN_U00 + (lane - 2)], u.v);
    else slot_put(slots, IN[VM_VOTE1_IN_U00 + (lane - 2)], u.v);
  } else if (HIN && lane >= 10 && lane < 16) {
    Fp h;
    hc.ld(h, lane - 10, he);
    if constexpr (TABLE) slot_put(slots, IN[VM_VOTE_T1_IN_U00 + (lane - 10)], h.v);
    else slot_put(slots, IN[VM_VOTE1_IN_U00 + (lane - 10)], h.v);
  } else if (TABLE && lane >= 6 && lane < 9) {
    Fp v;
    Slab{const_cast<uint32_t*>(pk.planes), pk.cap}.ld(v, lane - 6, e);
    if constexpr (TABLE) slot_put(slots, IN[VM_VOTE_T1_IN_PK_X + (lane - 6)], v.v);
  }
  __syncthreads();
  vm::run(prog.code, nph, 64, lane, true, slots, cst, scalar, vm::Out{s.p, s.cap, i});
  if (lane == 0) {
    const uint32_t sf = hdr[0], pf = hdr[1];
    const uint32_t sg_bad = sf & 1, sg_inf = (sf >> 1) & 1, sg_xz = (sf >> 2) & 1;
    uint32_t sg_ok, sg_grp, h_inf, pk_ok = 1, pk_grp = 1;
    if constexpr (TABLE) {
      sg_ok = slot_flag_get(slots, OUT[VM_VOTE_T1_OUT_SIG_OK]);
      sg_grp = slot_flag_get(slots, OUT[VM_VOTE_T1_OUT_SIG_GRP]);
      h_inf = HIN ? *hinf_in : slot_flag_get(slots, OUT[VM_VOTE_T1_OUT_H_INF]);
    } else {
      pk_ok = slot_flag_get(slots, OUT[VM_VOTE1_OUT_PK_OK]);
      pk_grp = slot_flag_get(slots, OUT[VM_VOTE1_OUT_PK_GRP]);
      sg_ok = slot_flag_get(slots, OUT[VM_VOTE1_OUT_SIG_OK]);
      sg_grp = slot_flag_get(slots, OUT[VM_VOTE1_OUT_SIG_GRP]);
      h_inf = HIN ? *hinf_in : slot_flag_get(slots, OUT[VM_VOTE1_OUT_H_INF]);
    }
    if (!HIN && hinf_out) *hinf_out = h_inf;
    uint32_t kf = pf;
    if (!TABLE) {
      const uint32_t pk_bad = pf & 1, pk_inf = (pf >> 1) & 1, pk_xz = (pf >> 2) & 1;
      kf = (pk_bad || (!pk_inf && (!pk_ok || pk_xz))) ? PKF_PARSE : pk_inf ? PKF_INF : !pk_grp ? PKF_GRP : 0u;
    }
    int32_t c;
    if (kf & PKF_PARSE) c = OVH_ERR_PUBKEY;
    else if (sg_bad) c = BLST_BAD_ENCODING;
    else if (!sg_inf && !sg_ok) c = BLST_POINT_NOT_ON_CURVE;
    else if (!sg_inf && (sg_xz || !sg_grp)) c = BLST_POINT_NOT_IN_GROUP;
    else if (kf & PKF_INF) c = BLST_PK_IS_INFINITY;
    else if (kf & PKF_GRP) c = BLST_POINT_NOT_IN_GROUP;
    else if (h_inf || sg_inf) c = BLST_VERIFY_FAIL;
    else c = 0;
    *code = c;
  }
}

template <bool TABLE>
__global__ __launch_bounds__(64) void k_vm_vote1(VmDev prog, const uint32_t* __restrict__ cst_g,
                                                 const uint8_t* __restrict__ pk_bytes, PkSrc pk,
                                                 const uint8_t* __restrict__ sig, Slab s, int32_t* __restrict__ code,
                                                 uint32_t* __restrict__ hinf_out = nullptr) {
  const uint32_t e = TABLE && pk.idx ? (uint32_t)pk.idx[0] : 0u;
  if constexpr (TABLE)
    vote_wave<true>(prog, VM_VOTE_T1_NPHASES, VM_VOTE_T1_NSLOTS, VM_VOTE_T1_IN, VM_VOTE_T1_OUT, cst_g, pk_bytes, pk, e,
                    sig, s, 0, 1, code, Slab{nullptr, 0}, 0, nullptr, hinf_out);
  else
    vote_wave<false>(prog, VM_VOTE1_NPHASES, VM_VOTE1_NSLOTS, VM_VOTE1_IN, VM_VOTE1_OUT, cst_g, pk_bytes, pk, e, sig,
                     s, 0, 1, code, Slab{nullptr, 0}, 0, nullptr, hinf_out);
}

template <bool TABLE>
__global__ __launch_bounds__(64) void k_vm_vote1h(VmDev prog, const uint32_t* __restrict__ cst_g,
                                                  const uint8_t* __restrict__ pk_bytes, PkSrc pk,
                                                  const uint8_t* __restrict__ sig, Slab s, int32_t* __restrict__ code,
                                                  Slab hc, uint32_t he, const uint32_t* __restrict__ hinf) {
  const uint32_t e = TABLE && pk.idx ? (uint32_t)pk.idx[0] : 0u;
  if constexpr (TABLE)
    vote_wave<true, true>(prog, VM_VOTE_T1H_NPHASES, VM_VOTE_T1H_NSLOTS, VM_VOTE_T1H_IN, VM_VOTE_T1H_OUT, cst_g,
                          pk_bytes, pk, e, sig, s, 0, 1, code, hc, he, hinf + he);
  else
    vote_wave<false, true>(prog, VM_VOTE1H_NPHASES, VM_VOTE1H_NSLOTS, VM_VOTE1H_IN, VM_VOTE1H_OUT, cst_g, pk_bytes, pk,
                           e, sig, s, 0, 1, code, hc, he, hinf + he);
}

__global__ __launch_bounds__(64) void k_copy_h(Slab s, Slab hc, uint32_t he) {
  for (uint32_t k = threadIdx.x; k < 6 * 12; k += 64) hc.p[(size_t)k * hc.cap + he] = s.p[(size_t)(S_RS * 12 + k) * s.cap];
}

template <bool TABLE>
__global__ __launch_bounds__(64) void k_vm_votew(uint32_t n, VmDev prog, const uint32_t* __restrict__ cst_g,
                                                 const uint8_t* __restrict__ pks, PkSrc pk,
                                                 const uint8_t* __restrict__ sigs, Slab s, uint64_t seed,
                                                 uint64_t base, int32_t* __restrict__ codes) {
  const uint32_t i = blockIdx.x;
  if (i >= n) return;
  const uint32_t e = TABLE ? (pk.idx ? (uint32_t)pk.idx[i] : i) : 0u;
  if constexpr (TABLE)
    vote_wave<true>(prog, VM_VOTEW_T_NPHASES, VM_VOTEW_T_NSLOTS, VM_VOTEW_T_IN, VM_VOTEW_T_OUT, cst_g, nullptr, pk, e,
                    sigs + (size_t)i * 96, s, i, vote_scalar(seed, base, i), codes + i);
  else
    vote_wave<false>(prog, VM_VOTEW_NPHASES, VM_VOTEW_NSLOTS, VM_VOTEW_IN, VM_VOTEW_OUT, cst_g, pks + (size_t)i * 48,
                     pk, e, sigs + (size_t)i * 96, s, i, vote_scalar(seed, base, i), codes + i);
}

constexpr uint32_t VSAME_NSLOTS = VM_VSAME_NSLOTS > VM_VSAME_T_NSLOTS ? VM_VSAME_NSLOTS : VM_VSAME_T_NSLOTS;
constexpr uint32_t VSAME_STRIDE_W = align256w(VSAME_NSLOTS * 12 + 4);
constexpr uint32_t VSAME8_NSLOTS = VM_VSAME8_NSLOTS > VM_VSAME8_T_NSLOTS ? VM_VSAME8_NSLOTS : VM_VSAME8_T_NSLOTS;
constexpr uint32_t VSAME8_STRIDE_W = align256w(VSAME8_NSLOTS * 12 + 4);
#ifndef VSAME8_MIN
#define VSAME8_MIN 2048u
#endif
constexpr uint32_t H2G_STRIDE_W = align256w(VM_H2G_NSLOTS * 12);
static_assert(VM_VSAME_W == 16 && VM_VSAME_T_W == 16 && VM_VSAME8_W == 8 && VM_VSAME8_T_W == 8 && VM_H2G_W == 16 && VM_GMIL_W == 64 && VM_H2G_NIN == 4 &&
                  VM_GMIL_NIN == 9 && VM_G_U == 0 && VM_G_PLANES == 22,
              "same-message program shapes (tools/fpvm/progs.py)");

#ifndef SM_PRIO
#define SM_PRIO 1
#endif
#ifndef SM_H2G_STREAMS
#define SM_H2G_STREAMS 3
#endif
static_assert(SM_H2G_STREAMS >= 1 && SM_H2G_STREAMS <= 4, "hstream[4]");
template <bool TABLE, uint32_t W = 16>
__global__ __launch_bounds__(64) void k_vm_vsame(uint32_t cnt, uint32_t lo, VmDev prog,
                                                 const uint32_t* __restrict__ cst_g, const uint8_t* __restrict__ pks,
                                                 PkSrc pk, const uint8_t* __restrict__ sigs, Slab s, uint64_t seed,
                                                 uint64_t base, int32_t* __restrict__ codes) {
  extern __shared__ uint4 lds4[];
  if (SM_PRIO) __builtin_amdgcn_s_setprio(2);
  uint32_t* lds = reinterpret_cast<uint32_t*>(lds4);
  uint32_t* cst = lds;
  static_assert(W == 16 || W == 8, "vsame slice width");
  constexpr bool W8 = W == 8;
  const uint32_t slice = threadIdx.x / W, lane = threadIdx.x % W;
  uint32_t* slots = lds + SLOT_BASE_W + slice * (W8 ? VSAME8_STRIDE_W : VSAME_STRIDE_W);
  constexpr uint32_t NS = W8 ? (TABLE ? VM_VSAME8_T_NSLOTS : VM_VSAME8_NSLOTS)
                             : (TABLE ? VM_VSAME_T_NSLOTS : VM_VSAME_NSLOTS);
  uint32_t* hdr = slots + NS * 12;
  const uint16_t* IN = W8 ? (TABLE ? VM_VSAME8_T_IN : VM_VSAME8_IN) : (TABLE ? VM_VSAME_T_IN : VM_VSAME_IN);
  const uint16_t* OUT = W8 ? (TABLE ? VM_VSAME8_T_OUT : VM_VSAME8_OUT) : (TABLE ? VM_VSAME_T_OUT : VM_VSAME_OUT);
  const uint32_t j = blockIdx.x * (64 / W) + slice, i = lo + j;
  const bool active = j < cnt;
  load_consts(cst, cst_g, VM_NCONST);
  if (active) {
    if (lane == 0) {
      uint32_t x1[12], x0[12], bad, inf, sort, xz;
      parse_hdr(sigs + (size_t)j * 96, 96, x1, x0, bad, inf, sort, xz);
      slot_put(slots, IN[TABLE ? VM_VSAME_T_IN_SIG_X1 : VM_VSAME_IN_SIG_X1], x1);
      slot_put(slots, IN[TABLE ? VM_VSAME_T_IN_SIG_X0 : VM_VSAME_IN_SIG_X0], x0);
      slot_flag(slots, IN[TABLE ? VM_VSAME_T_IN_SIG_SORT : VM_VSAME_IN_SIG_SORT], sort);
      hdr[0] = bad | inf << 1 | xz << 2;
    } else if (lane == 1) {
      if constexpr (TABLE) {
        hdr[1] = pk.flags[pk.idx[j]];
      } else {
        uint32_t x[12], bad, inf, sort, xz;
        parse_hdr(pks + (size_t)j * 48, 48, x, x, bad, inf, sort, xz);
        slot_put(slots, IN[VM_VSAME_IN_PK_X], x);
        slot_flag(slots, IN[VM_VSAME_IN_PK_SORT], sort);
        hdr[1] = bad | inf << 1 | xz << 2;
      }
    } else if (TABLE && lane >= 2 && lane < 5) {
      Fp v;
      Slab{const_cast<uint32_t*>(pk.planes), pk.cap}.ld(v, lane - 2, (uint32_t)pk.idx[j]);
      slot_put(slots, IN[VM_VSAME_T_IN_PK_X + (lane - 2)], v.v);
    }
  }
  __syncthreads();
  constexpr uint32_t NPH = W8 ? (TABLE ? VM_VSAME8_T_NPHASES : VM_VSAME8_NPHASES)
                              : (TABLE ? VM_VSAME_T_NPHASES : VM_VSAME_NPHASES);
  vm::run(prog.code, NPH, W, lane, active, slots, cst, vote_scalar(seed, base, i), vm::Out{s.p, s.cap, i});
  if (active && lane == 0) {
    const uint32_t sf = hdr[0], pf = hdr[1];
    const uint32_t sg_bad = sf & 1, sg_inf = (sf >> 1) & 1, sg_xz = (sf >> 2) & 1;
    uint32_t kf = pf, sg_ok, sg_grp;
    if constexpr (TABLE) {
      sg_ok = slot_flag_get(slots, OUT[VM_VSAME_T_OUT_SIG_OK]);
      sg_grp = slot_flag_get(slots, OUT[VM_VSAME_T_OUT_SIG_GRP]);
    } else {
      sg_ok = slot_flag_get(slots, OUT[VM_VSAME_OUT_SIG_OK]);
      sg_grp = slot_flag_get(slots, OUT[VM_VSAME_OUT_SIG_GRP]);
      const uint32_t pk_ok = slot_flag_get(slots, OUT[VM_VSAME_OUT_PK_OK]);
      const uint32_t pk_grp = slot_flag_get(slots, OUT[VM_VSAME_OUT_PK_GRP]);
      const uint32_t pk_bad = pf & 1, pk_inf = (pf >> 1) & 1, pk_xz = (pf >> 2) & 1;
      kf = (pk_bad || (!pk_inf && (!pk_ok || pk_xz))) ? PKF_PARSE : pk_inf ? PKF_INF : !pk_grp ? PKF_GRP : 0u;
    }
    int32_t c;
    if (kf & PKF_PARSE) c = OVH_ERR_PUBKEY;
    else if (sg_bad) c = BLST_BAD_ENCODING;
    else if (!sg_inf && !sg_ok) c = BLST_POINT_NOT_ON_CURVE;
    else if (!sg_inf && (sg_xz || !sg_grp)) c = BLST_POINT_NOT_IN_GROUP;
    else if (kf & PKF_INF) c = BLST_PK_IS_INFINITY;
    else if (kf & PKF_GRP) c = BLST_POINT_NOT_IN_GROUP;
    else if (sg_inf) c = BLST_VERIFY_FAIL;
    else c = 0;
    codes[i] = c;
  }
}

__global__ __launch_bounds__(64) void k_vm_h2g(uint32_t G, VmDev prog, const uint32_t* __restrict__ cst_g, Slab g,
                                               uint32_t* __restrict__ ghinf) {
  extern __shared__ uint4 lds4[];
  if (SM_PRIO) __builtin_amdgcn_s_setprio(3);
  uint32_t* lds = reinterpret_cast<uint32_t*>(lds4);
  uint32_t* cst = lds;
  const uint32_t slice = threadIdx.x / 16, lane = threadIdx.x % 16;
  uint32_t* slots = lds + SLOT_BASE_W + slice * H2G_STRIDE_W;
  const uint32_t q = blockIdx.x * VM_SLICES + slice;
  const bool active = q < G;
  load_consts(cst, cst_g, VM_NCONST);
  if (active && lane < 4) {
    Fp u;
    g.ld(u, VM_G_U + lane, q);
    slot_put(slots, VM_H2G_IN[lane], u.v);
  }
  __syncthreads();
  vm::run(prog.code, VM_H2G_NPHASES, 16, lane, active, slots, cst, 0, vm::Out{g.p, g.cap, q});
  if (active && lane == 0) ghinf[q] = slot_flag_get(slots, VM_H2G_OUT[VM_H2G_OUT_H_INF]) ? 1u : 0u;
}

__global__ __launch_bounds__(WG) void k_samemsg_fix(uint32_t n, const uint32_t* __restrict__ gid,
                                                    const uint32_t* __restrict__ ghinf, int32_t* __restrict__ codes,
                                                    Slab P) {
  const uint32_t i = blockIdx.x * WG + threadIdx.x;
  if (i >= n) return;
  int32_t c = codes[i];
  if (c == 0 && ghinf[gid[i]]) codes[i] = c = BLST_VERIFY_FAIL;
  if (c != 0) {
    Fp z, o;
    fp_zero(z);
    fp_one(o);
    P.st(z, 0, i);
    P.st(o, 1, i);
    P.st(z, 2, i);
  }
}

__global__ __launch_bounds__(64) void k_vm_g1pairs(uint32_t npairs, VmDev prog, uint32_t stride_w,
                                                   const uint32_t* __restrict__ cst_g, const uint32_t* __restrict__ pairs,
                                                   Slab P) {
  constexpr uint32_t W = VM_G1PADD_W, SL = 64 / W;
  extern __shared__ uint4 lds4[];
  uint32_t* lds = reinterpret_cast<uint32_t*>(lds4);
  uint32_t* cst = lds;
  const uint32_t slice = threadIdx.x / W, lane = threadIdx.x % W;
  uint32_t* slots = lds + SLOT_BASE_W + slice * stride_w;
  const uint32_t q = blockIdx.x * SL + slice;
  const bool active = q < npairs;
  const uint32_t a = active ? pairs[2 * q] : 0u, b = active ? pairs[2 * q + 1] : 0u;
  load_consts(cst, cst_g, VM_NCONST);
  if (active) {
    for (uint32_t k = lane; k < 6; k += W) {
      Fp v;
      P.ld(v, k % 3, k < 3 ? a : b);
      slot_put(slots, prog.in[k], v.v);
    }
  }
  __syncthreads();
  vm::run(prog.code, prog.nphases, W, lane, active, slots, cst, 0, vm::Out{nullptr, 0, 0});
  if (active) {
    for (uint32_t k = lane; k < 3; k += W) {
      Fp v;
      const uint32_t src = prog.out[k];
      for (int l = 0; l < 12; ++l) v.v[l] = slots[src * 12 + l];
      vm::canon(v, v);
      P.st(v, k, a);
    }
  }
}

__global__ __launch_bounds__(64) void k_pick_head(uint32_t G, const uint32_t* __restrict__ head, Slab P,
                                                  const uint32_t* __restrict__ ghinf, uint32_t* __restrict__ sel) {
  uint32_t best = 0xFFFFFFFFu;
  for (uint32_t q = threadIdx.x; q < G; q += 64) {
    Fp z;
    P.ld(z, 2, head[q]);
    if (!fp_is_zero(z) && !ghinf[q] && q < best) best = q;
  }
  for (uint32_t off = 32; off; off >>= 1) {
    const uint32_t o = __shfl_xor(best, off);
    best = o < best ? o : best;
  }
  if (threadIdx.x == 0) *sel = best == 0xFFFFFFFFu ? 0u : best;
}

__global__ __launch_bounds__(64) void k_vm_gmil(uint32_t G, const uint32_t* __restrict__ sel, VmDev prog,
                                                const uint32_t* __restrict__ cst_g, const uint32_t* __restrict__ head,
                                                Slab P, Slab g) {
  extern __shared__ uint4 lds4[];
  uint32_t* lds = reinterpret_cast<uint32_t*>(lds4);
  uint32_t* cst = lds;
  uint32_t* slots = lds + SLOT_BASE_W;
  __shared__ uint32_t zinf;
  const uint32_t hsel = *sel;
  const uint32_t q = blockIdx.x, lane = threadIdx.x;
  if (q >= G || q == hsel) return;
  const uint32_t oq = q == 0 ? hsel : q;
  const uint32_t a = head[q];
  load_consts(cst, cst_g, VM_NCONST);
  if (lane == 0) {
    Fp z;
    P.ld(z, 2, a);
    zinf = fp_is_zero(z) ? 1u : 0u;
  }
  if (lane < 9) {
    Fp v;
    if (lane < 3) P.ld(v, lane, a);
    else g.ld(v, VM_G_H + (lane - 3), q);
    slot_put(slots, VM_GMIL_IN[lane], v.v);
  }
  __syncthreads();
  if (zinf) {
    if (lane < 12) {
      Fp v;
      if (lane == 0) fp_one(v);
      else fp_zero(v);
      g.st(v, VM_G_F + lane, oq);
    }
    return;
  }
  vm::run(prog.code, VM_GMIL_NPHASES, 64, lane, true, slots, cst, 0, vm::Out{g.p, g.cap, oq});
}

template <bool TABLE>
__global__ __launch_bounds__(64) void k_vm_vote1h_b(uint32_t cnt, uint32_t lo, VmDev prog,
                                                    const uint32_t* __restrict__ cst_g,
                                                    const uint8_t* __restrict__ pks, PkSrc pk,
                                                    const uint8_t* __restrict__ sigs, Slab s, int32_t* __restrict__ codes,
                                                    const uint32_t* __restrict__ gid, Slab gH,
                                                    const uint32_t* __restrict__ ghinf,
                                                    const int32_t* __restrict__ verdict) {
  if (*verdict == 1) return;
  const uint32_t j = blockIdx.x, i = lo + j;
  if (j >= cnt || codes[i] != 0) return;
  const uint32_t e = TABLE ? (uint32_t)pk.idx[j] : 0u;
  if constexpr (TABLE)
    vote_wave<true, true>(prog, VM_VOTE_T1H_NPHASES, VM_VOTE_T1H_NSLOTS, VM_VOTE_T1H_IN, VM_VOTE_T1H_OUT, cst_g,
                          nullptr, pk, e, sigs + (size_t)j * 96, s, i, 1, codes + i, gH, gid[i], ghinf + gid[i]);
  else
    vote_wave<false, true>(prog, VM_VOTE1H_NPHASES, VM_VOTE1H_NSLOTS, VM_VOTE1H_IN, VM_VOTE1H_OUT, cst_g,
                           pks + (size_t)j * 48, pk, e, sigs + (size_t)j * 96, s, i, 1, codes + i, gH, gid[i],
                           ghinf + gid[i]);
}

static_assert(VM_GFIN_W == 64 && VM_GFIN_NIN == 27, "gfin inputs: F, apk, H, S");
__global__ __launch_bounds__(64) void k_vm_gfin(VmDev prog, const uint32_t* __restrict__ cst_g, Slab F,
                                                const uint32_t* __restrict__ head, const uint32_t* __restrict__ sel,
                                                Slab P, Slab gH, Slab S, int32_t* __restrict__ verdict) {
  extern __shared__ uint4 lds4[];
  if (SM_PRIO) __builtin_amdgcn_s_setprio(3);
  uint32_t* lds = reinterpret_cast<uint32_t*>(lds4);
  uint32_t* cst = lds;
  uint32_t* slots = lds + SLOT_BASE_W;
  __shared__ uint32_t degenerate;
  const uint32_t lane = threadIdx.x, hsel = *sel, a = head[hsel];
  load_consts(cst, cst_g, VM_NCONST);
  if (lane == 0) {
    Fp za, zs;
    P.ld(za, 2, a);
    S.ld(zs, 4, 0);
    Fp zs1;
    S.ld(zs1, 5, 0);
    degenerate = (fp_is_zero(za) || (fp_is_zero(zs) && fp_is_zero(zs1))) ? 1u : 0u;
  }
  if (lane < 27) {
    Fp v;
    if (lane < 12) {
      if (F.p) F.ld(v, lane, 0);
      else if (lane == 0) fp_one(v);
      else fp_zero(v);
    } else if (lane < 15) {
      P.ld(v, lane - 12, a);
    } else if (lane < 21) {
      gH.ld(v, lane - 15, hsel);
    } else {
      S.ld(v, lane - 21, 0);
    }
    slot_put(slots, VM_GFIN_IN[lane], v.v);
  }
  __syncthreads();
  if (degenerate) {
    if (lane == 0) *verdict = 0;
    return;
  }
  vm::run(prog.code, VM_GFIN_NPHASES, 64, lane, true, slots, cst, 0, vm::Out{nullptr, 0, 0});
  if (lane == 0) *verdict = slot_flag_get(slots, VM_GFIN_OUT[0]) ? 1 : 0;
}

__global__ __launch_bounds__(64) void k_vm_qcpre(VmDev prog, const uint32_t* __restrict__ cst_g,
                                                 const uint8_t* __restrict__ sig, Slab s, uint32_t* __restrict__ flags) {
  extern __shared__ uint4 lds4[];
  uint32_t* lds = reinterpret_cast<uint32_t*>(lds4);
  uint32_t* cst = lds;
  uint32_t* slots = lds + SLOT_BASE_W;
  uint32_t* hdr = slots + VM_QCPRE_NSLOTS * 12;
  const uint32_t lane = threadIdx.x;
  load_consts(cst, cst_g, VM_NCONST);
  if (lane == 0) {
    uint32_t x1[12], x0[12], bad, inf, sort, xz;
    parse_hdr(sig, 96, x1, x0, bad, inf, sort, xz);
    slot_put(slots, VM_QCPRE_IN[VM_QCPRE_IN_SIG_X1], x1);
    slot_put(slots, VM_QCPRE_IN[VM_QCPRE_IN_SIG_X0], x0);
    slot_flag(slots, VM_QCPRE_IN[VM_QCPRE_IN_SIG_SORT], sort);
    hdr[0] = bad | inf << 1 | xz << 2;
  } else if (lane >= 2 && lane < 6) {
    Fp u;
    s.ld(u, S_U + (lane - 2), 0);
    slot_put(slots, VM_QCPRE_IN[VM_QCPRE_IN_U00 + (lane - 2)], u.v);
  }
  __syncthreads();
  vm::run(prog.code, VM_QCPRE_NPHASES, VM_QCPRE_W, lane, true, slots, cst, 0, vm::Out{s.p, s.cap, 0});
  if (lane == 0)
    *flags = hdr[0] | slot_flag_get(slots, VM_QCPRE_OUT[VM_QCPRE_OUT_SIG_OK]) << 8 |
             slot_flag_get(slots, VM_QCPRE_OUT[VM_QCPRE_OUT_SIG_GRP]) << 9 |
             slot_flag_get(slots, VM_QCPRE_OUT[VM_QCPRE_OUT_H_INF]) << 10;
}

__global__ __launch_bounds__(64) void k_vm_qcmil(VmDev prog, const uint32_t* __restrict__ cst_g, PkSrc pk, Slab s,
                                                 const uint32_t* __restrict__ flags, int32_t* __restrict__ code) {
  extern __shared__ uint4 lds4[];
  uint32_t* lds = reinterpret_cast<uint32_t*>(lds4);
  uint32_t* cst = lds;
  uint32_t* slots = lds + SLOT_BASE_W;
  const uint32_t lane = threadIdx.x;
  load_consts(cst, cst_g, VM_NCONST);
  if (lane < 21) {
    Fp v;
    if (lane < 3) Slab{const_cast<uint32_t*>(pk.planes), pk.cap}.ld(v, lane, 0);
    else if (lane < 9) s.ld(v, S_RS + (lane - 3), 0);
    else s.ld(v, S_F + (lane - 9), 0);
    slot_put(slots, VM_QCMIL_IN[lane], v.v);
  }
  __syncthreads();
  vm::run(prog.code, VM_QCMIL_NPHASES, VM_QCMIL_W, lane, true, slots, cst, 0, vm::Out{s.p, s.cap, 1});
  if (lane == 0) {
    const uint32_t sf = *flags, kf = pk.flags[0];
    const uint32_t sg_bad = sf & 1, sg_inf = (sf >> 1) & 1, sg_xz = (sf >> 2) & 1;
    const uint32_t sg_ok = (sf >> 8) & 1, sg_grp = (sf >> 9) & 1, h_inf = (sf >> 10) & 1;
    int32_t c;
    if (kf & PKF_PARSE) c = OVH_ERR_PUBKEY;
    else if (sg_bad) c = BLST_BAD_ENCODING;
    else if (!sg_inf && !sg_ok) c = BLST_POINT_NOT_ON_CURVE;
    else if (!sg_inf && (sg_xz || !sg_grp)) c = BLST_POINT_NOT_IN_GROUP;
    else if (kf & PKF_INF) c = BLST_PK_IS_INFINITY;
    else if (kf & PKF_GRP) c = BLST_POINT_NOT_IN_GROUP;
    else if (h_inf || sg_inf) c = BLST_VERIFY_FAIL;
    else c = 0;
    *code = c;
  }
}
static_assert(VM_QCMIL_NIN == 21 && VM_QCPRE_W == 64 && VM_QCMIL_W == 64, "qcmil inputs: apk X Y Z, H, g");

__device__ __forceinline__ bool fe_one(const VmDev& prog, const uint32_t* __restrict__ cst_g, Slab F, uint32_t u) {
  extern __shared__ uint4 lds4[];
  uint32_t* lds = reinterpret_cast<uint32_t*>(lds4);
  uint32_t* cst = lds;
  uint32_t* slots = lds + SLOT_BASE_W;
  const uint32_t lane = threadIdx.x;
  load_consts(cst, cst_g, VM_NCONST);
  if (lane < 12) {
    Fp v;
    F.ld(v, lane, u);
    slot_put(slots, VM_FINAL1_IN[lane], v.v);
  }
  __syncthreads();
  vm::run(prog.code, VM_FINAL1_NPHASES, VM_FINAL1_W, lane, true, slots, cst, 0, vm::Out{nullptr, 0, 0});
  return slot_flag_get(slots, VM_FINAL1_OUT[0]) != 0;
}

__global__ __launch_bounds__(64) void k_vm_fe(VmDev prog, const uint32_t* __restrict__ cst_g, Slab F,
                                              int32_t* __restrict__ verdict) {
  const bool ok = fe_one(prog, cst_g, F, 0);
  if (threadIdx.x == 0) *verdict = ok ? 1 : 0;
}

__global__ __launch_bounds__(64) void k_vm_votefe(uint32_t n, VmDev prog, const uint32_t* __restrict__ cst_g, Slab s,
                                                  int32_t* __restrict__ codes, const int32_t* __restrict__ verdict) {
  if (*verdict == 1) return;
  const uint32_t i = blockIdx.x;
  if (i >= n || codes[i] != 0) return;
  const bool ok = fe_one(prog, cst_g, Slab{s.p + (size_t)S_F * 12 * s.cap, s.cap}, i);
  if (threadIdx.x == 0) codes[i] = ok ? 0 : BLST_VERIFY_FAIL;
}

__global__ __launch_bounds__(64) void k_vm_final1(VmDev prog, const uint32_t* __restrict__ cst_g, Slab F,
                                                  int32_t* __restrict__ code, int32_t* __restrict__ verdict) {
  if (*code != 0) {
    if (threadIdx.x == 0) *verdict = 0;
    return;
  }
  const bool ok = fe_one(prog, cst_g, F, 0);
  if (threadIdx.x == 0) {
    *verdict = ok ? 1 : 0;
    if (!ok) *code = BLST_VERIFY_FAIL;
  }
}

__device__ __forceinline__ bool final_one(uint32_t u, const VmDev& prog, const uint32_t* __restrict__ cst_g, Slab inF,
                                          Slab inS) {
  extern __shared__ uint4 lds4[];
  uint32_t* lds = reinterpret_cast<uint32_t*>(lds4);
  uint32_t* cst = lds;
  uint32_t* slots = lds + SLOT_BASE_W;
  const uint32_t lane = threadIdx.x;
  load_consts(cst, cst_g, VM_NCONST);
  for (uint32_t k = lane; k < 4 * PART_PLANES; k += 64) {
    const uint32_t q = k / PART_PLANES, j = k % PART_PLANES;
    Fp v;
    if (q == 0) {
      if (j < 12) inF.ld(v, j, u);
      else inS.ld(v, j - 12, u);
    } else if (j == 0 || j == 12 + 2) {
      fp_one(v);
    } else {
      fp_zero(v);
    }
    slot_put(slots, VM_FINAL_IN[k], v.v);
  }
  __syncthreads();
  vm::run(prog.code, VM_FINAL_NPHASES, VM_FINAL_W, lane, true, slots, cst, 0, vm::Out{nullptr, 0, 0});
  return slot_flag_get(slots, VM_FINAL_OUT[0]) != 0;
}

#define GROUP_VOTES 16
__global__ __launch_bounds__(64) void k_vm_group(uint32_t m, VmDev prog, const uint32_t* __restrict__ cst_g, Slab inF,
                                                 Slab inS, const int32_t* __restrict__ verdict,
                                                 int32_t* __restrict__ grp_ok) {
  if (verdict && *verdict == 1) return;
  const uint32_t g = blockIdx.x;
  if (g >= m) return;
  const bool ok = final_one(g, prog, cst_g, inF, inS);
  if (threadIdx.x == 0) grp_ok[g] = ok ? 1 : 0;
}

__global__ __launch_bounds__(64) void k_vm_votechk(uint32_t n, VmDev prog, const uint32_t* __restrict__ cst_g, Slab s,
                                                   int32_t* __restrict__ codes, const int32_t* __restrict__ verdict,
                                                   const int32_t* __restrict__ grp_ok) {
  if (verdict && *verdict == 1) return;
  const uint32_t i = blockIdx.x;
  if (i >= n || codes[i] != 0 || grp_ok[i / GROUP_VOTES]) return;
  const bool ok = final_one(i, prog, cst_g, Slab{s.p + (size_t)S_F * 12 * s.cap, s.cap},
                            Slab{s.p + (size_t)S_RS * 12 * s.cap, s.cap});
  if (threadIdx.x == 0) codes[i] = ok ? 0 : BLST_VERIFY_FAIL;
}

constexpr uint32_t RS_STRIDE_W = align256w(VM_RS_NSLOTS * 12);
__global__ __launch_bounds__(64) void k_vm_rs(uint32_t n, VmDev prog, const uint32_t* __restrict__ cst_g, Slab s,
                                              uint64_t seed, uint64_t base, const int32_t* __restrict__ codes,
                                              const int32_t* __restrict__ verdict) {
  if (verdict && *verdict == 1) return;
  extern __shared__ uint4 lds4[];
  uint32_t* lds = reinterpret_cast<uint32_t*>(lds4);
  uint32_t* cst = lds;
  const uint32_t slice = threadIdx.x / VM_RS_W, lane = threadIdx.x % VM_RS_W;
  uint32_t* slots = lds + SLOT_BASE_W + slice * RS_STRIDE_W;
  const uint32_t i = blockIdx.x * (64 / VM_RS_W) + slice;
  const bool active = i < n && codes[i] == 0;
  load_consts(cst, cst_g, VM_NCONST);
  if (active && lane < VM_RS_NIN) {
    Fp v;
    s.ld(v, (lane < 4 ? S_SIG : S_TAU - 4) + lane, i);
    slot_put(slots, VM_RS_IN[lane], v.v);
  }
  __syncthreads();
  vm::run(prog.code, VM_RS_NPHASES, VM_RS_W, lane, active, slots, cst, vote_scalar(seed, base, i),
          vm::Out{s.p, s.cap, i});
}

#define GROUPCHECK_FAIL (0x100 | BLST_POINT_NOT_IN_GROUP)
constexpr uint32_t SIGCHK_STRIDE_W = align256w(VM_SIGCHK_NSLOTS * 12 + 4);
__global__ __launch_bounds__(64) void k_vm_sigchk(uint32_t n, VmDev prog, const uint32_t* __restrict__ cst_g,
                                                  const uint8_t* __restrict__ data, const uint64_t* __restrict__ off,
                                                  int gc, int32_t* __restrict__ codes, Slab pts) {
  extern __shared__ uint4 lds4[];
  uint32_t* lds = reinterpret_cast<uint32_t*>(lds4);
  uint32_t* cst = lds;
  const uint32_t slice = threadIdx.x / VM_SIGCHK_W, lane = threadIdx.x % VM_SIGCHK_W;
  uint32_t* slots = lds + SLOT_BASE_W + slice * SIGCHK_STRIDE_W;
  uint32_t* hdr = slots + VM_SIGCHK_NSLOTS * 12;
  const uint32_t i = blockIdx.x * (64 / VM_SIGCHK_W) + slice;
  const bool active = i < n;
  load_consts(cst, cst_g, VM_NCONST);
  if (active && lane == 0) {
    uint32_t x1[12], x0[12], bad, inf, sort, xz;
    parse_hdr(data + off[i], 96, x1, x0, bad, inf, sort, xz);
    slot_put(slots, VM_SIGCHK_IN[VM_SIGCHK_IN_SIG_X1], x1);
    slot_put(slots, VM_SIGCHK_IN[VM_SIGCHK_IN_SIG_X0], x0);
    slot_flag(slots, VM_SIGCHK_IN[VM_SIGCHK_IN_SIG_SORT], sort);
    hdr[0] = bad | inf << 1 | xz << 2;
  }
  __syncthreads();
  vm::run(prog.code, VM_SIGCHK_NPHASES, VM_SIGCHK_W, lane, active, slots, cst, 0, vm::Out{nullptr, 0, 0});
  __syncthreads();
  if (!active) return;
  const uint32_t pf = hdr[0];
  int32_t c = BLST_SUCCESS;
  bool pt = false;
  if (pf & 1) {
    c = BLST_BAD_ENCODING;
  } else if (!(pf & 2)) {
    if (!slot_flag_get(slots, VM_SIGCHK_OUT[VM_SIGCHK_OUT_SIG_OK])) c = BLST_POINT_NOT_ON_CURVE;
    else if (gc && ((pf & 4) || !slot_flag_get(slots, VM_SIGCHK_OUT[VM_SIGCHK_OUT_SIG_GRP]))) c = GROUPCHECK_FAIL;
    else pt = true;
  }
  for (uint32_t k = lane; k < 6; k += VM_SIGCHK_W) {
    Fp v;
    if (pt && k < 4) {
      const uint32_t src = VM_SIGCHK_OUT[VM_SIGCHK_OUT_Q0 + k];
      for (int l = 0; l < 12; ++l) v.v[l] = slots[src * 12 + l];
      vm::canon(v, v);
    } else if (k == (pt ? 4u : 2u)) {
      fp_one(v);
    } else {
      fp_zero(v);
    }
    pts.st(v, k, i);
  }
  if (lane == 0) codes[i] = c;
}

__global__ __launch_bounds__(64) void k_vm_g2tree(uint32_t m, VmDev prog, uint32_t stride_w,
                                                  const uint32_t* __restrict__ cst_g, Slab in, Slab out) {
  constexpr uint32_t W = VM_PADD_W, SL = 64 / W;
  extern __shared__ uint4 lds4[];
  uint32_t* lds = reinterpret_cast<uint32_t*>(lds4);
  uint32_t* cst = lds;
  const uint32_t slice = threadIdx.x / W, lane = threadIdx.x % W;
  uint32_t* slots = lds + SLOT_BASE_W + slice * stride_w;
  const uint32_t q = blockIdx.x * SL + slice;
  const bool active = q < (m + 1) / 2;
  load_consts(cst, cst_g, VM_NCONST);
  if (active) {
    for (uint32_t k = lane; k < 12; k += W) {
      const uint32_t e = 2 * q + k / 6, c = k % 6;
      Fp v;
      if (e < m) in.ld(v, c, e);
      else if (c == 2) fp_one(v);
      else fp_zero(v);
      slot_put(slots, prog.in[k], v.v);
    }
  }
  __syncthreads();
  vm::run(prog.code, prog.nphases, W, lane, active, slots, cst, 0, vm::Out{nullptr, 0, 0});
  if (active) {
    for (uint32_t k = lane; k < 6; k += W) {
      Fp v;
      const uint32_t src = prog.out[k];
      for (int l = 0; l < 12; ++l) v.v[l] = slots[src * 12 + l];
      vm::canon(v, v);
      out.st(v, k, q);
    }
  }
}

__global__ __launch_bounds__(64) void k_g2p_compress(Slab in, uint8_t* out) {
  if (threadIdx.x) return;
  Fp2 X, Y, Z, zz;
  in.ld2(X, 0, 0);
  in.ld2(Y, 2, 0);
  in.ld2(Z, 4, 0);
  G2J j;
  fp2_mul(j.X, X, Z);
  fp2_sqr(zz, Z);
  fp2_mul(j.Y, Y, zz);
  j.Z = Z;
  g2_compress(out, j);
}

constexpr uint32_t PKGEN_STRIDE_W = align256w(VM_PKGEN_NSLOTS * 12 + 3 * 12);
__global__ __launch_bounds__(64) void k_vm_pkgen(uint32_t n, VmDev prog, const uint32_t* __restrict__ cst_g,
                                                 const uint8_t* __restrict__ sks, uint8_t* __restrict__ out, Slab bl) {
  static_assert(VM_PKGEN_NIN == 3 && VM_PKGEN_NOUT == 3, "pkgen program shape (tools/fpvm/progs.py)");
  constexpr uint32_t W = VM_PKGEN_W;
  extern __shared__ uint4 lds4[];
  uint32_t* lds = reinterpret_cast<uint32_t*>(lds4);
  uint32_t* cst = lds;
  const uint32_t slice = threadIdx.x / W, lane = threadIdx.x % W;
  uint32_t* slots = lds + SLOT_BASE_W + slice * PKGEN_STRIDE_W;
  uint32_t* acc = slots + VM_PKGEN_NSLOTS * 12;
  const uint32_t i = blockIdx.x * (64 / W) + slice;
  const bool active = i < n;
  load_consts(cst, cst_g, VM_NCONST);
  uint64_t k[4] = {0, 0, 0, 0};
  if (active) {
    const uint8_t* b = sks + (size_t)i * 32;
    for (int j = 0; j < 4; ++j)
      for (int t = 0; t < 8; ++t) k[j] = k[j] << 8 | b[8 * j + t];
    if (lane < 3)
      for (int l = 0; l < 12; ++l) acc[lane * 12 + l] = lane == 1 ? ONE_M[l] : 0u;
  }
  __syncthreads();
  for (int r = 0; r < 4; ++r) {
    if (active && lane < 3) slot_put(slots, VM_PKGEN_IN[lane], acc + lane * 12);
    __syncthreads();
    vm::run(prog.code, VM_PKGEN_NPHASES, W, lane, active, slots, cst, k[r], vm::Out{nullptr, 0, 0});
    __syncthreads();
    if (active && lane < 3) {
      Fp t;
      for (int l = 0; l < 12; ++l) t.v[l] = slots[VM_PKGEN_OUT[lane] * 12 + l];
      vm::canon(t, t);
      for (int l = 0; l < 12; ++l) acc[lane * 12 + l] = t.v[l];
    }
    __syncthreads();
  }
  k[0] = k[1] = k[2] = k[3] = 0;
  if (active && lane == 0) {
    Fp X, Y, Z, zz, beta;
    for (int l = 0; l < 12; ++l) {
      X.v[l] = acc[l];
      Y.v[l] = acc[12 + l];
      Z.v[l] = acc[24 + l];
    }
    bl.ld(beta, 0, i);
    fp_mul(X, X, beta);
    fp_mul(Y, Y, beta);
    fp_mul(Z, Z, beta);
    G1J j;
    fp_mul(j.X, X, Z);
    fp_sqr(zz, Z);
    fp_mul(j.Y, Y, zz);
    j.Z = Z;
    g1_compress(out + (size_t)i * 48, j);
  }
}

constexpr uint64_t X_ABS64 = 0xD201000000010000ull;
constexpr uint64_t R64[4] = {0xFFFFFFFF00000001ull, 0x53BDA402FFFE5BFEull, 0x3339D80809A1D805ull,
                             0x73EDA753299D7D48ull};
__device__ __forceinline__ void gls_digits(uint64_t d[4], uint64_t n[4]) {
  for (int rep = 0; rep < 2; ++rep) {
    uint64_t t[4], br = 0;
    for (int l = 0; l < 4; ++l) {
      const uint64_t a = n[l], b = R64[l];
      const uint64_t d1 = a - b;
      const uint64_t b1 = (uint64_t)(a < b);
      t[l] = d1 - br;
      br = b1 | (uint64_t)(d1 < br);
    }
    const uint64_t keep = 0ull - br;
    for (int l = 0; l < 4; ++l) n[l] = (n[l] & keep) | (t[l] & ~keep);
  }
  for (int i = 0; i < 3; ++i) {
    uint64_t rem = 0;
    for (int l = 3; l >= 0; --l) {
      uint64_t q = 0;
      for (int b = 63; b >= 0; --b) {
        const uint64_t top = rem >> 63;
        rem = (rem << 1) | ((n[l] >> b) & 1u);
        const uint64_t ge = top | (uint64_t)(rem >= X_ABS64);
        rem -= X_ABS64 & (0ull - ge);
        q |= ge << b;
      }
      n[l] = q;
    }
    d[i] = rem;
  }
  d[3] = n[0];
}

__device__ __forceinline__ uint64_t signg_scalar(const uint64_t d[4], int j) {
  uint64_t v = 0;
  for (int t = 0; t < 16; ++t)
    for (int i = 0; i < 4; ++i) v |= ((d[i] >> (48 - 16 * j + t)) & 1ull) << (4 * t + i);
  return v;
}

constexpr uint32_t SIGNG_NSLOTS = VM_SIGNG0_NSLOTS > VM_SIGNG1_NSLOTS ? VM_SIGNG0_NSLOTS : VM_SIGNG1_NSLOTS;
constexpr uint32_t SIGNG_STRIDE_W = align256w(SIGNG_NSLOTS * 12 + 96 * 12 + 8);
__global__ __launch_bounds__(64) void k_vm_signg(uint32_t n, VmDev p0, VmDev p1, const uint32_t* __restrict__ cst_g,
                                                 const uint8_t* __restrict__ sks, Slab s, uint8_t* __restrict__ out,
                                                 Slab bl) {
  static_assert(VM_SIGNG0_W == VM_SIGNG1_W && VM_SIGNG0_NOUT == 96 && VM_SIGNG1_NIN == 96 && VM_SIGNG1_NOUT == 6,
                "signg program shapes (tools/fpvm/progs.py)");
  constexpr uint32_t W = VM_SIGNG0_W;
  extern __shared__ uint4 lds4[];
  uint32_t* lds = reinterpret_cast<uint32_t*>(lds4);
  uint32_t* cst = lds;
  const uint32_t slice = threadIdx.x / W, lane = threadIdx.x % W;
  uint32_t* slots = lds + SLOT_BASE_W + slice * SIGNG_STRIDE_W;
  uint32_t* hst = slots + SIGNG_NSLOTS * 12;
  uint64_t* dig = reinterpret_cast<uint64_t*>(hst + 96 * 12);
  const uint32_t i = blockIdx.x * (64 / W) + slice;
  const bool active = i < n;
  load_consts(cst, cst_g, VM_NCONST);
  if (active) {
    if (lane == 0) {
      const uint8_t* b = sks + (size_t)i * 32;
      uint64_t k[4] = {0, 0, 0, 0}, d[4];
      for (int j = 0; j < 4; ++j)
        for (int t = 0; t < 8; ++t) k[3 - j] = k[3 - j] << 8 | b[8 * j + t];
      gls_digits(d, k);
      for (int j = 0; j < 4; ++j) dig[j] = d[j];
      k[0] = k[1] = k[2] = k[3] = 0;
      d[0] = d[1] = d[2] = d[3] = 0;
    } else if (lane >= 1 && lane < 5) {
      Fp u;
      s.ld(u, S_U + (lane - 1), i);
      slot_put(slots, VM_SIGNG0_IN[lane - 1], u.v);
    }
  }
  __syncthreads();
  uint64_t d[4] = {0, 0, 0, 0};
  if (active)
    for (int j = 0; j < 4; ++j) d[j] = dig[j];
  vm::run(p0.code, VM_SIGNG0_NPHASES, W, lane, active, slots, cst, signg_scalar(d, 0), vm::Out{nullptr, 0, 0});
  __syncthreads();
  if (active)
    for (uint32_t q = lane; q < 96; q += W)
      for (int l = 0; l < 12; ++l) hst[q * 12 + l] = slots[VM_SIGNG0_OUT[q] * 12 + l];
  __syncthreads();
  for (int r = 1; r < 4; ++r) {
    if (active)
      for (uint32_t q = lane; q < 96; q += W) slot_put(slots, VM_SIGNG1_IN[q], hst + q * 12);
    __syncthreads();
    vm::run(p1.code, VM_SIGNG1_NPHASES, W, lane, active, slots, cst, signg_scalar(d, r), vm::Out{nullptr, 0, 0});
    __syncthreads();
    if (active && lane < 6)
      for (int l = 0; l < 12; ++l) hst[lane * 12 + l] = slots[VM_SIGNG1_OUT[lane] * 12 + l];
    __syncthreads();
  }
  d[0] = d[1] = d[2] = d[3] = 0;
  if (active && lane < 4) dig[lane] = 0;
  if (active && lane < 6) {
    Fp t;
    for (int l = 0; l < 12; ++l) t.v[l] = hst[lane * 12 + l];
    vm::canon(t, t);
    for (int l = 0; l < 12; ++l) hst[lane * 12 + l] = t.v[l];
  }
  __syncthreads();
  if (active && lane == 0) {
    Fp2 X, Y, Z, zz;
    for (int l = 0; l < 12; ++l) {
      X.c0.v[l] = hst[l];
      X.c1.v[l] = hst[12 + l];
      Y.c0.v[l] = hst[24 + l];
      Y.c1.v[l] = hst[36 + l];
      Z.c0.v[l] = hst[48 + l];
      Z.c1.v[l] = hst[60 + l];
    }
    Fp2 beta;
    bl.ld2(beta, 0, i);
    fp2_mul(X, X, beta);
    fp2_mul(Y, Y, beta);
    fp2_mul(Z, Z, beta);
    G2J j;
    fp2_mul(j.X, X, Z);
    fp2_sqr(zz, Z);
    fp2_mul(j.Y, Y, zz);
    j.Z = Z;
    g2_compress(out + (size_t)i * 96, j);
  }
}

#include "msm.hpp"
#include "qc.hpp"

constexpr uint32_t PKCHK_STRIDE_W = align256w(VM_PKCHK_NSLOTS * 12 + 4);
__global__ __launch_bounds__(64) void k_vm_pkchk(uint32_t n, VmDev prog, const uint32_t* __restrict__ cst_g,
                                                 const uint8_t* __restrict__ pks, Slab pts, uint32_t* __restrict__ flags) {
  extern __shared__ uint4 lds4[];
  uint32_t* lds = reinterpret_cast<uint32_t*>(lds4);
  uint32_t* cst = lds;
  const uint32_t slice = threadIdx.x / VM_PKCHK_W, lane = threadIdx.x % VM_PKCHK_W;
  uint32_t* slots = lds + SLOT_BASE_W + slice * PKCHK_STRIDE_W;
  uint32_t* hdr = slots + VM_PKCHK_NSLOTS * 12;
  const uint32_t i = blockIdx.x * (64 / VM_PKCHK_W) + slice;
  const bool active = i < n;
  load_consts(cst, cst_g, VM_NCONST);
  if (active && lane == 0) {
    uint32_t x[12], bad, inf, sort, xz;
    parse_hdr(pks + (size_t)i * 48, 48, x, x, bad, inf, sort, xz);
    slot_put(slots, VM_PKCHK_IN[VM_PKCHK_IN_PK_X], x);
    slot_flag(slots, VM_PKCHK_IN[VM_PKCHK_IN_PK_SORT], sort);
    hdr[0] = bad | inf << 1 | xz << 2;
  }
  __syncthreads();
  vm::run(prog.code, VM_PKCHK_NPHASES, VM_PKCHK_W, lane, active, slots, cst, 0, vm::Out{nullptr, 0, 0});
  __syncthreads();
  if (!active) return;
  const uint32_t pf = hdr[0];
  uint32_t f = 0;
  if ((pf & 1) || (!(pf & 2) && (!slot_flag_get(slots, VM_PKCHK_OUT[VM_PKCHK_OUT_PK_OK]) || (pf & 4)))) f = PKF_PARSE;
  else if (pf & 2) f = PKF_INF;
  else if (!slot_flag_get(slots, VM_PKCHK_OUT[VM_PKCHK_OUT_PK_GRP])) f = PKF_GRP;
  const bool pt = f == 0 || f == PKF_GRP;
  for (uint32_t k = lane; k < 3; k += VM_PKCHK_W) {
    Fp v;
    if (pt && k < 2) {
      const uint32_t src = VM_PKCHK_OUT[VM_PKCHK_OUT_P0 + k];
      for (int l = 0; l < 12; ++l) v.v[l] = slots[src * 12 + l];
      vm::canon(v, v);
    } else if (k == (pt ? 2u : 1u)) {
      fp_one(v);
    } else {
      fp_zero(v);
    }
    pts.st(v, k, i);
  }
  if (lane == 0) flags[i] = f;
}

__global__ __launch_bounds__(64) void k_vm_g1tree(uint32_t m, VmDev prog, uint32_t stride_w,
                                                  const uint32_t* __restrict__ cst_g, Slab in, Slab out) {
  constexpr uint32_t W = VM_G1PADD_W, SL = 64 / W;
  extern __shared__ uint4 lds4[];
  uint32_t* lds = reinterpret_cast<uint32_t*>(lds4);
  uint32_t* cst = lds;
  const uint32_t slice = threadIdx.x / W, lane = threadIdx.x % W;
  uint32_t* slots = lds + SLOT_BASE_W + slice * stride_w;
  const uint32_t q = blockIdx.x * SL + slice;
  const bool active = q < (m + 1) / 2;
  load_consts(cst, cst_g, VM_NCONST);
  if (active) {
    for (uint32_t k = lane; k < 6; k += W) {
      const uint32_t e = 2 * q + k / 3, c = k % 3;
      Fp v;
      if (e < m) in.ld(v, c, e);
      else if (c == 1) fp_one(v);
      else fp_zero(v);
      slot_put(slots, prog.in[k], v.v);
    }
  }
  __syncthreads();
  vm::run(prog.code, prog.nphases, W, lane, active, slots, cst, 0, vm::Out{nullptr, 0, 0});
  if (active) {
    for (uint32_t k = lane; k < 3; k += W) {
      Fp v;
      const uint32_t src = prog.out[k];
      for (int l = 0; l < 12; ++l) v.v[l] = slots[src * 12 + l];
      vm::canon(v, v);
      out.st(v, k, q);
    }
  }
}

__global__ __launch_bounds__(64) void k_apk_finish(Slab in, Slab out, uint32_t* __restrict__ flags) {
  const uint32_t k = threadIdx.x;
  if (k >= 3) return;
  Fp v;
  in.ld(v, k, 0);
  out.st(v, k, 0);
  if (k == 2) {
    uint32_t z = 0;
    for (int l = 0; l < 12; ++l) z |= v.v[l];
    flags[0] = z ? 0u : PKF_INF;
  }
}

constexpr uint32_t G1GRP_STRIDE_W = align256w(VM_G1GRP_NSLOTS * 12);
__global__ __launch_bounds__(64) void k_vm_g1grp(VmDev prog, const uint32_t* __restrict__ cst_g, Slab apk,
                                                 uint32_t* __restrict__ flags) {
  extern __shared__ uint4 lds4[];
  uint32_t* lds = reinterpret_cast<uint32_t*>(lds4);
  uint32_t* cst = lds;
  const uint32_t slice = threadIdx.x / VM_G1GRP_W, lane = threadIdx.x % VM_G1GRP_W;
  uint32_t* slots = lds + SLOT_BASE_W;
  const bool active = slice == 0;
  load_consts(cst, cst_g, VM_NCONST);
  if (active && lane < 3) {
    Fp v;
    apk.ld(v, lane, 0);
    slot_put(slots, VM_G1GRP_IN[lane], v.v);
  }
  __syncthreads();
  vm::run(prog.code, VM_G1GRP_NPHASES, VM_G1GRP_W, lane, active, slots, cst, 0, vm::Out{nullptr, 0, 0});
  if (active && lane == 0 && !(flags[0] & PKF_INF) && !slot_flag_get(slots, VM_G1GRP_OUT[VM_G1GRP_OUT_PK_GRP]))
    flags[0] |= PKF_GRP;
}

__global__ __launch_bounds__(64) void k_qc_apk(uint32_t nq, const uint32_t* __restrict__ off,
                                               const uint32_t* __restrict__ ent, Slab table, Slab out,
                                               uint32_t* __restrict__ flags) {
  __shared__ uint32_t red[64 * 36];
  const uint32_t q = blockIdx.x, t = threadIdx.x;
  if (q >= nq) return;
  G1J acc, x;
  jac_set_inf(acc);
  for (uint32_t k = off[q] + t; k < off[q + 1]; k += 64) {
    const uint32_t e = ent[k];
    table.ld(x.X, 0, e);
    table.ld(x.Y, 1, e);
    table.ld(x.Z, 2, e);
    jac_add(acc, acc, x);
  }
  for (uint32_t s = 32; s >= 1; s >>= 1) {
    if (t >= s && t < 2 * s) {
      for (int l = 0; l < 12; ++l) {
        red[(t - s) * 36 + l] = acc.X.v[l];
        red[(t - s) * 36 + 12 + l] = acc.Y.v[l];
        red[(t - s) * 36 + 24 + l] = acc.Z.v[l];
      }
    }
    __syncthreads();
    if (t < s) {
      for (int l = 0; l < 12; ++l) {
        x.X.v[l] = red[t * 36 + l];
        x.Y.v[l] = red[t * 36 + 12 + l];
        x.Z.v[l] = red[t * 36 + 24 + l];
      }
      jac_add(acc, acc, x);
    }
    __syncthreads();
  }
  if (t) return;
  Fp X, Y, Z;
  uint32_t f = 0;
  if (jac_is_inf(acc)) {
    fp_zero(X);
    fp_one(Y);
    fp_zero(Z);
    f = PKF_INF;
  } else {
    Fp zz;
    fp_mul(X, acc.X, acc.Z);
    Y = acc.Y;
    fp_sqr(zz, acc.Z);
    fp_mul(Z, zz, acc.Z);
  }
  out.st(X, 0, q);
  out.st(Y, 1, q);
  out.st(Z, 2, q);
  flags[q] = f;
}

__global__ __launch_bounds__(64) void k_unpack_partials(uint32_t k, const uint32_t* __restrict__ parts, Slab F, Slab S) {
  const uint32_t t = blockIdx.x * 64 + threadIdx.x;
  if (t >= k * PART_PLANES) return;
  const uint32_t q = t / PART_PLANES, j = t % PART_PLANES;
  Fp v;
  for (int l = 0; l < 12; ++l) v.v[l] = parts[(size_t)q * 216 + j * 12 + l];
  if (j < 12) F.st(v, j, q);
  else S.st(v, j - 12, q);
}

__global__ __launch_bounds__(64) void k_pack_partial2(Slab F, Slab S, uint32_t* __restrict__ out) {
  const uint32_t t = threadIdx.x;
  if (t >= PART_PLANES) return;
  Fp v;
  if (t < 12) F.ld(v, t, 0);
  else S.ld(v, t - 12, 0);
  for (int l = 0; l < 12; ++l) out[t * 12 + l] = v.v[l];
}

__device__ __noinline__ void canon_sig(const uint8_t* __restrict__ sig, uint32_t sl, uint8_t* __restrict__ sig96) {
  if (sl == 96 && (sig[0] & 0x80)) {
    for (int i = 0; i < 96; ++i) sig96[i] = sig[i];
    return;
  }
  G2A a;
  bool inf;
  const int e = g2_from_bytes(a, inf, sig, sl);
  for (int i = 0; i < 96; ++i) sig96[i] = 0;
  if (e == BLST_SUCCESS && inf) {
    sig96[0] = 0xc0;
  } else if (e == BLST_SUCCESS || e == BLST_POINT_NOT_IN_GROUP) {
    fp_to_be48(sig96, a.x.c1);
    fp_to_be48(sig96 + 48, a.x.c0);
    sig96[0] |= 0x80 | (fp2_lex_largest(a.y) ? 0x20 : 0);
  } else if (e == BLST_POINT_NOT_ON_CURVE) {
    sig96[0] = 0x80;
    sig96[95] = 1;
  } else {
    sig96[0] = 0x9f;
    for (int i = 1; i < 96; ++i) sig96[i] = 0xff;
  }
}

__device__ __noinline__ void canon_pk(const uint8_t* __restrict__ pk, uint32_t pl, uint8_t* __restrict__ pk48) {
  if (pl == 48 && (pk[0] & 0x80)) {
    for (int i = 0; i < 48; ++i) pk48[i] = pk[i];
    return;
  }
  G1A a;
  bool inf;
  const int e = g1_from_bytes(a, inf, pk, pl);
  for (int i = 0; i < 48; ++i) pk48[i] = 0;
  if (e == BLST_SUCCESS && inf) {
    pk48[0] = 0xc0;
  } else if (e == BLST_SUCCESS) {
    fp_to_be48(pk48, a.x);
    pk48[0] |= 0x80 | (fp_lex_largest(a.y) ? 0x20 : 0);
  } else {
    pk48[0] = 0x9f;
    for (int i = 1; i < 48; ++i) pk48[i] = 0xff;
  }
}

__global__ __launch_bounds__(64) void k_canon_one(const uint8_t* __restrict__ sig, uint32_t sl,
                                                  const uint8_t* __restrict__ pk, uint32_t pl, uint8_t* __restrict__ sig96,
                                                  uint8_t* __restrict__ pk48) {
  if (threadIdx.x != 0) return;
  canon_sig(sig, sl, sig96);
  canon_pk(pk, pl, pk48);
}

__global__ __launch_bounds__(WG) void k_canon_qc(uint32_t n, const uint8_t* __restrict__ data,
                                                 const uint64_t* __restrict__ off, const uint64_t* __restrict__ len,
                                                 const uint8_t* __restrict__ sig, uint32_t sl, uint8_t* __restrict__ out) {
  const uint32_t i = blockIdx.x * WG + threadIdx.x;
  if (i < n) canon_pk(data + off[i], (uint32_t)len[i], out + (size_t)48 * i);
  if (i == n) canon_sig(sig, sl, out + (size_t)48 * n);
}

__global__ __launch_bounds__(WG) void k_canon_sig_list(uint32_t n, const uint8_t* __restrict__ data,
                                                       const uint64_t* __restrict__ off, const uint64_t* __restrict__ len,
                                                       uint8_t* __restrict__ out, uint64_t* __restrict__ offs) {
  const uint32_t i = blockIdx.x * WG + threadIdx.x;
  if (i >= n) return;
  canon_sig(data + off[i], (uint32_t)len[i], out + (size_t)96 * i);
  offs[i] = (uint64_t)96 * i;
}

__global__ __launch_bounds__(WG) void k_parse_pk_list(uint32_t n, const uint8_t* __restrict__ data,
                                                      const uint64_t* __restrict__ off, const uint64_t* __restrict__ len,
                                                      int32_t* __restrict__ codes, Slab pts) {
  const uint32_t i = blockIdx.x * WG + threadIdx.x;
  if (i >= n) return;
  G1A a;
  bool inf;
  int e = g1_from_bytes(a, inf, data + off[i], (uint32_t)len[i]);
  Fp X, Y, Z;
  if (e == BLST_SUCCESS && !inf) {
    X = a.x;
    Y = a.y;
    fp_one(Z);
  } else {
    fp_one(X);
    fp_one(Y);
    fp_zero(Z);
  }
  pts.st(X, 0, i);
  pts.st(Y, 1, i);
  pts.st(Z, 2, i);
  codes[i] = e;
}

constexpr uint32_t PKDEC_STRIDE_W = align128w(VM_PKDEC_NSLOTS * 12 + 4);
__global__ __launch_bounds__(64) void k_vm_pkdec(uint32_t n, VmDev prog, const uint32_t* __restrict__ cst_g,
                                                 const uint8_t* __restrict__ data, const uint64_t* __restrict__ off,
                                                 int32_t* __restrict__ codes) {
  constexpr uint32_t W = VM_PKDEC_W, SL = 64 / W;
  extern __shared__ uint4 lds4[];
  uint32_t* lds = reinterpret_cast<uint32_t*>(lds4);
  uint32_t* cst = lds;
  const uint32_t slice = threadIdx.x / W, lane = threadIdx.x % W;
  uint32_t* slots = lds + SLOT_BASE_W + slice * PKDEC_STRIDE_W;
  uint32_t* hdr = slots + VM_PKDEC_NSLOTS * 12;
  const uint32_t i = blockIdx.x * SL + slice;
  const bool active = i < n;
  load_consts(cst, cst_g, VM_NCONST);
  if (active && lane == 0) {
    uint32_t x[12], bad, inf, sort, xz;
    parse_hdr(data + off[i], 48, x, x, bad, inf, sort, xz);
    slot_put(slots, VM_PKDEC_IN[VM_PKCHK_IN_PK_X], x);
    slot_flag(slots, VM_PKDEC_IN[VM_PKCHK_IN_PK_SORT], sort);
    hdr[0] = bad | inf << 1 | xz << 2;
  }
  __syncthreads();
  vm::run(prog.code, VM_PKDEC_NPHASES, W, lane, active, slots, cst, 0, vm::Out{nullptr, 0, 0});
  if (active && lane == 0) {
    const uint32_t pf = hdr[0];
    int32_t c = BLST_SUCCESS;
    if (pf & 1) c = BLST_BAD_ENCODING;
    else if (!(pf & 2) && !slot_flag_get(slots, VM_PKDEC_OUT[VM_PKDEC_OUT_PK_OK])) c = BLST_POINT_NOT_ON_CURVE;
    else if (!(pf & 2) && (pf & 4)) c = BLST_POINT_NOT_IN_GROUP;
    codes[i] = c;
  }
}

__global__ __launch_bounds__(WG) void k_sum_g1(uint32_t n, Slab pts, uint32_t* out_jac , uint8_t* out48) {
  if (threadIdx.x != 0 || blockIdx.x != 0) return;
  G1J acc, x;
  jac_set_inf(acc);
  for (uint32_t i = 0; i < n; ++i) {
    pts.ld(x.X, 0, i);
    pts.ld(x.Y, 1, i);
    pts.ld(x.Z, 2, i);
    jac_add(acc, acc, x);
  }
  for (int k = 0; k < 12; ++k) {
    out_jac[k] = acc.X.v[k];
    out_jac[12 + k] = acc.Y.v[k];
    out_jac[24 + k] = acc.Z.v[k];
  }
  if (out48) g1_compress(out48, acc);
}

__global__ __launch_bounds__(WG) void k_verify_agg(const uint32_t* agg_pk_jac, const uint8_t* sig, uint32_t sl, const uint8_t* hash,
                             uint32_t hl, XmdTemplates t, int32_t* out) {
  if (threadIdx.x != 0 || blockIdx.x != 0) return;
  G2A s;
  bool sinf;
  int e = g2_from_bytes(s, sinf, sig, sl);
  if (e != BLST_SUCCESS) {
    *out = e;
    return;
  }
  if (hl != 32) {
    *out = OVH_ERR_HASH_LEN;
    return;
  }
  G1J pj;
  for (int k = 0; k < 12; ++k) {
    pj.X.v[k] = agg_pk_jac[k];
    pj.Y.v[k] = agg_pk_jac[12 + k];
    pj.Z.v[k] = agg_pk_jac[24 + k];
  }
  G1A pa;
  bool pinf = !jac_to_aff(pa, pj);
  uint32_t msg[8];
  be_words_from_bytes(msg, hash, 8);
  *out = core_verify(pa, pinf, s, sinf, msg, t);
}

__device__ void sk_words(uint32_t k[8], const uint8_t* sk) {
  for (int i = 0; i < 8; ++i) {
    const uint8_t* p = sk + 28 - 4 * i;
    k[i] = ((uint32_t)p[0] << 24) | ((uint32_t)p[1] << 16) | ((uint32_t)p[2] << 8) | p[3];
  }
}

struct ValidatorTable {
  uint32_t n = 0, cap = 0;
  uint32_t* planes = nullptr;
  uint32_t* flags = nullptr;
  uint32_t* qc = nullptr;
  std::vector<uint32_t> hflags;
  std::vector<std::string> keys;
  std::unordered_map<std::string, uint32_t> index;
  std::vector<uint32_t> sorted;
};

struct VerdictCache {
  std::mutex mu;
  std::unordered_map<std::string, int32_t> map;
  std::deque<std::string> fifo;
  size_t cap = 1u << 16;
  uint64_t hits = 0, misses = 0;
};

struct HostBatch {
  int32_t* codes = nullptr;
  size_t n = 0;
  int ring = 0;
  struct Dev {
    size_t d, lo, cnt;
    std::vector<uint32_t> perm;
  };
  std::vector<Dev> dev;
};

#define NFIN_STREAMS 4u
struct ovh_ctx {
  int device = 0;
  uint32_t flags = 0;
  hipStream_t stream = nullptr;
  hipStream_t fstream = nullptr, fstream2 = nullptr, fstream3 = nullptr;
  hipStream_t fstream4 = nullptr;
  uint32_t nfin = NFIN_STREAMS;
  hipStream_t xstream = nullptr;
  hipStream_t vstream[3] = {};
  hipStream_t hstream[4] = {};
  hipStream_t pool_st[3] = {};
  uint64_t* pool_q = nullptr;
  void* pool_desc = nullptr;
  uint32_t* pool_scr = nullptr;
  uint32_t pool_wgs = 0;
  uint32_t pool_grid0 = 0;
  uint32_t ncu = 256;
  uint32_t pool_rsv = 0;
  uint32_t pool_ncu = 256;
  uint64_t pool_seq = 0;
  uint32_t* pool_err = nullptr;
  uint64_t* plog = nullptr;
  uint64_t plog_seq[OVH_BATCH_SLOTS] = {};
  uint64_t plog_grids = 0;
  hipStream_t fs[OVH_BATCH_SLOTS] = {};
  hipEvent_t ev_front[OVH_BATCH_SLOTS] = {}, ev_back[OVH_BATCH_SLOTS] = {};
  hipEvent_t ev_x[4] = {};
  uint32_t* state_slot[OVH_BATCH_SLOTS] = {};
  uint32_t* red_slot[OVH_BATCH_SLOTS] = {};
  uint32_t *state_all = nullptr, *red_all = nullptr;
  uint8_t* pstage_all = nullptr;
  size_t state_w = 0, red_w = 0, pstage_b = 0;
  int32_t* grp_ok[OVH_BATCH_SLOTS] = {};
  uint32_t slot_n[OVH_BATCH_SLOTS] = {};
  uint32_t* fin = nullptr;
  uint32_t pipe_k = 0;
  int last_slot = 0;
  uint32_t small_max = SMALL_MAX;
  XmdTemplates xmd;
  std::mutex mu;
  uint32_t cap = 0, red_cap = 0;
  uint8_t* in_buf = nullptr;
  size_t in_cap = 0;
  uint32_t* scr = nullptr;
  int32_t *scr_pk = nullptr, *scr_sig = nullptr;
  uint32_t scr_cap = 0;
  uint32_t* comb = nullptr;
  uint32_t comb_cap = 0;
  uint32_t* part_out = nullptr;
  int32_t* result = nullptr;
  uint32_t last_n = 0;
  uint64_t test_seed = 0, test_base = 0;
  ValidatorTable tab;
  uint32_t* qc_buf = nullptr;
  uint32_t qc_cap = 0;
  uint32_t* qt_buf = nullptr;
  uint32_t qt_cap = 0;
  VerdictCache cache;
  std::vector<ovh_ctx*> sub;
  std::atomic<uint32_t> rr{0};
  std::vector<uint8_t> peer;
  std::vector<int> fin_devs;
  uint8_t* gather = nullptr;
  uint32_t* mfin = nullptr;
  uint32_t* msm_buf[OVH_BATCH_SLOTS] = {};
  uint64_t slot_seed[OVH_BATCH_SLOTS] = {}, slot_base[OVH_BATCH_SLOTS] = {};
  uint8_t* hst_h[OVH_BATCH_SLOTS] = {};
  uint8_t* hst_d[OVH_BATCH_SLOTS] = {};
  size_t hst_cap[OVH_BATCH_SLOTS] = {};
  hipEvent_t ev_m[OVH_BATCH_SLOTS][4] = {};
  uint8_t* mg = nullptr;
  std::deque<HostBatch> hq;
  uint64_t hb_k = 0;
  VmDev vm_vsame{}, vm_vsame_t{}, vm_vsame8{}, vm_vsame8_t{}, vm_h2g{}, vm_gmil{}, vm_pkdec{}, vm_g1grp{}, vm_gfin{};
  uint32_t* gslab[OVH_BATCH_SLOTS] = {};
  uint32_t gcap[OVH_BATCH_SLOTS] = {};
  int samemsg = 1;
  uint32_t shard_span = 0;
  uint32_t shard_streams = 2;
  uint8_t* pstage[OVH_BATCH_SLOTS] = {};
  uint64_t sm_batches = 0, sm_votes = 0, sm_hashes = 0;
  uint32_t* sm1_plan = nullptr;
  size_t sm1_n = 0;
  std::vector<uint32_t> sm1_lo;
  uint8_t* sm1_hash = nullptr;
  VmDev vm_vote{}, vm_vote_t{}, vm_fold{}, vm_final{}, vm_rs{}, vm_madd{}, vm_padd{}, vm_hdbl[5]{}, vm_sigchk{},
      vm_pkchk{}, vm_g1padd{}, vm_vote1{}, vm_vote_t1{}, vm_final1{}, vm_votew{},
      vm_votew_t{}, vm_qcpre{}, vm_qcmil{}, vm_vote1h{}, vm_vote_t1h{}, vm_pkgen{}, vm_signg0{}, vm_signg1{};
  uint32_t* hc_planes = nullptr;
  uint32_t* hc_inf = nullptr;
  std::unordered_map<std::string, uint32_t> hc_index;
  std::vector<std::string> hc_keys;
  uint32_t hc_next = 0;
  uint64_t hc_hits = 0, hc_misses = 0;
  uint32_t* vm_consts = nullptr;
  std::vector<void*> vm_bufs;
  uint32_t clk_wgs = 0;
  bool clk_table = false;
  std::vector<uint32_t> blind_h;
  hipEvent_t ev0[OVH_NSTAGES] = {}, ev1[OVH_NSTAGES] = {};
  static constexpr uint32_t VEV_CAP = 256;
  hipEvent_t vev0[VEV_CAP] = {}, vev1[VEV_CAP] = {};
  uint32_t vev_n = 0;
  uint32_t ev_mask = 0;
};

#define HIPCHK(x)                                  \
  do {                                             \
    if ((x) != hipSuccess) return OVH_ERR_DEVICE;  \
  } while (0)
#define CHK(x)                \
  do {                              \
    const int e_ = (x);             \
    if (e_) return e_;              \
  } while (0)

static const char* const STAGE_NAMES[OVH_NSTAGES] = {"hash_to_field", "vote", "fold", "final", "bisect", "msm"};

static constexpr size_t LDS_VOTE = ((size_t)SLOT_BASE_W + VM_SLICES * (size_t)VOTE_STRIDE_W) * 4;
static constexpr size_t LDS_VOTE_T = ((size_t)SLOT_BASE_W + VM_SLICES * (size_t)VOTE_T_STRIDE_W) * 4;
static constexpr size_t LDS_FOLD = ((size_t)SLOT_BASE_W + VM_FOLD_UNITS * (size_t)FOLD_STRIDE_W) * 4;
static constexpr size_t LDS_FINAL = ((size_t)SLOT_BASE_W + (size_t)VM_FINAL_NSLOTS * 12) * 4;
static_assert(VM_VOTE_W * VM_SLICES == 64 && VM_VOTE_T_W * VM_SLICES == 64 && VM_FOLD_W * VM_FOLD_UNITS == 64 &&
                  VM_FINAL_W == 64, "VM slice widths");
static constexpr size_t LDS_FOLD1 = ((size_t)SLOT_BASE_W + (size_t)FOLD_STRIDE_W) * 4;
static constexpr size_t LDS_RS = ((size_t)SLOT_BASE_W + (64 / VM_RS_W) * (size_t)RS_STRIDE_W) * 4;
constexpr uint32_t cmax(uint32_t a, uint32_t b) { return a > b ? a : b; }
static constexpr uint32_t MSM8_STRIDE_W = align128w(cmax(VM_MADD_NSLOTS, VM_PADD_NSLOTS) * 12);
static constexpr uint32_t HDBL_STRIDE_W =
    align128w(cmax(cmax(cmax(VM_HDBL1_NSLOTS, VM_HDBL2_NSLOTS), cmax(VM_HDBL4_NSLOTS, VM_HDBL8_NSLOTS)), VM_HDBL16_NSLOTS) * 12);
static constexpr size_t LDS_MSM8 = ((size_t)SLOT_BASE_W + (64 / VM_MADD_W) * (size_t)MSM8_STRIDE_W) * 4;
static constexpr size_t LDS_HDBL = ((size_t)SLOT_BASE_W + (64 / VM_HDBL1_W) * (size_t)HDBL_STRIDE_W) * 4;
static_assert(VM_MADD_W == VM_PADD_W && VM_HDBL1_W == VM_HDBL2_W && VM_HDBL1_W == VM_HDBL4_W && VM_HDBL1_W == VM_HDBL8_W &&
                  VM_HDBL1_W == VM_HDBL16_W && VM_MADD_NIN == 10 && VM_PADD_NIN == 12 && VM_HDBL1_NIN == 12,
              "MSM program shapes (tools/fpvm/progs.py)");
static constexpr size_t LDS_SIGCHK = ((size_t)SLOT_BASE_W + (64 / VM_SIGCHK_W) * (size_t)SIGCHK_STRIDE_W) * 4;
static constexpr uint32_t VOTE1_NSLOTS = VM_VOTE1_NSLOTS > VM_VOTE_T1_NSLOTS ? VM_VOTE1_NSLOTS : VM_VOTE_T1_NSLOTS;
static constexpr size_t LDS_VOTE1 = ((size_t)SLOT_BASE_W + VOTE1_NSLOTS * 12 + 4) * 4;
static constexpr uint32_t VOTE1H_NSLOTS = VM_VOTE1H_NSLOTS > VM_VOTE_T1H_NSLOTS ? VM_VOTE1H_NSLOTS : VM_VOTE_T1H_NSLOTS;
static constexpr size_t LDS_VOTE1H = ((size_t)SLOT_BASE_W + VOTE1H_NSLOTS * 12 + 4) * 4;
static constexpr uint32_t VOTEW_NSLOTS = VM_VOTEW_NSLOTS > VM_VOTEW_T_NSLOTS ? VM_VOTEW_NSLOTS : VM_VOTEW_T_NSLOTS;
static constexpr size_t LDS_VOTEW = ((size_t)SLOT_BASE_W + VOTEW_NSLOTS * 12 + 4) * 4;
static constexpr size_t LDS_QCPRE = ((size_t)SLOT_BASE_W + VM_QCPRE_NSLOTS * 12 + 4) * 4;
static constexpr size_t LDS_QCMIL = ((size_t)SLOT_BASE_W + VM_QCMIL_NSLOTS * 12) * 4;
static constexpr size_t LDS_FINAL1 = ((size_t)SLOT_BASE_W + (size_t)VM_FINAL1_NSLOTS * 12) * 4;
static constexpr size_t LDS_SIGNG = ((size_t)SLOT_BASE_W + (64 / VM_SIGNG0_W) * (size_t)SIGNG_STRIDE_W) * 4;
static_assert(LDS_SIGNG <= 80 * 1024, "signg LDS (raised limit, ovh_create)");
static constexpr size_t LDS_PKGEN = ((size_t)SLOT_BASE_W + (64 / VM_PKGEN_W) * (size_t)PKGEN_STRIDE_W) * 4;
static constexpr size_t LDS_PKCHK = ((size_t)SLOT_BASE_W + (64 / VM_PKCHK_W) * (size_t)PKCHK_STRIDE_W) * 4;
static constexpr uint32_t G1PADD_STRIDE_W = align128w(VM_G1PADD_NSLOTS * 12);
static constexpr size_t LDS_G1PADD = ((size_t)SLOT_BASE_W + (64 / VM_G1PADD_W) * (size_t)G1PADD_STRIDE_W) * 4;
static_assert(LDS_RS <= 64 * 1024 && LDS_MSM8 <= 64 * 1024 && LDS_HDBL <= 64 * 1024 && LDS_SIGCHK <= 64 * 1024 &&
                  LDS_PKCHK <= 64 * 1024 && LDS_G1PADD <= 64 * 1024 && LDS_PKGEN <= 64 * 1024 &&
                  LDS_VOTE1 <= 64 * 1024 && LDS_FINAL1 <= 64 * 1024 && LDS_VOTEW <= 64 * 1024 && LDS_QCPRE <= 64 * 1024 && LDS_VOTE1H <= 64 * 1024 &&
                  LDS_QCMIL <= 64 * 1024 && VM_G1PADD_NIN == 6,
              "default LDS limit");
static_assert(LDS_VOTE <= 160 * 1024 && LDS_VOTE_T <= 160 * 1024 && LDS_FINAL <= 160 * 1024, "VM LDS budget");
static constexpr size_t LDS_VSAME = ((size_t)SLOT_BASE_W + VM_SLICES * (size_t)VSAME_STRIDE_W) * 4;
static constexpr size_t LDS_VSAME8 = ((size_t)SLOT_BASE_W + 8 * (size_t)VSAME8_STRIDE_W) * 4;
static_assert(LDS_VSAME8 <= 64 * 1024, "vsame8 LDS (default limit)");
static constexpr size_t LDS_H2G = ((size_t)SLOT_BASE_W + VM_SLICES * (size_t)H2G_STRIDE_W) * 4;
static constexpr size_t LDS_GMIL = ((size_t)SLOT_BASE_W + (size_t)VM_GMIL_NSLOTS * 12) * 4;
static_assert(LDS_VSAME <= 64 * 1024 && LDS_H2G <= 64 * 1024 && LDS_GMIL + 16 <= 64 * 1024, "same-message LDS");
static constexpr size_t LDS_PKDEC = ((size_t)SLOT_BASE_W + (64 / VM_PKDEC_W) * (size_t)PKDEC_STRIDE_W) * 4;
static_assert(LDS_PKDEC <= 64 * 1024 && VM_PKDEC_NIN == 2, "pkdec LDS / shape");
static constexpr size_t LDS_G1GRP = ((size_t)SLOT_BASE_W + (size_t)G1GRP_STRIDE_W) * 4;
static_assert(LDS_G1GRP <= 64 * 1024 && VM_G1GRP_NIN == 3, "g1grp LDS / shape");
static constexpr size_t LDS_GFIN = ((size_t)SLOT_BASE_W + (size_t)VM_GFIN_NSLOTS * 12) * 4;
static_assert(LDS_GFIN + 16 <= 64 * 1024, "gfin LDS");
constexpr size_t lds_granule(size_t b) { return (b + 1023) / 1024 * 1024; }
static constexpr size_t LDS_POOL = LDS_VOTE > LDS_VOTE_T ? LDS_VOTE : LDS_VOTE_T;
static_assert(8 * lds_granule(LDS_POOL) <= 160 * 1024, "eight pool workgroups per CU");
static_assert(VOTE_NSCR <= 4096 && VM_VOTE_NSLOTS <= 2048 && VM_VOTE_T_NSLOTS <= 2048,
              "side words: 12-bit scratch entries, 11-bit slots (fpvm.hpp side_spill)");
#ifndef POOL_HOLES_PER_8CU
#define POOL_HOLES_PER_8CU 8u
#endif
#define POOL_MAX_WGS 4096u
static_assert(FOLD_STRIDE_W <= VM_SLICES * VOTE_STRIDE_W && FOLD_STRIDE_W <= VM_SLICES * VOTE_T_STRIDE_W,
              "fused fold reuses the vote slots");

static int vm_upload(ovh_ctx* c, VmDev& d, const uint32_t* code, uint32_t nphases, uint32_t W, uint32_t NW,
                     const uint16_t* in, uint32_t nin, const uint16_t* out, uint32_t nout,
                     const uint32_t* side = nullptr) {
  const size_t words = (size_t)nphases * W * NW, pad = (size_t)vm::PREFETCH * W * NW;
  void *dc = nullptr, *di = nullptr, *dout = nullptr;
  HIPCHK(hipMalloc(&dc, (words + pad) * 4));
  c->vm_bufs.push_back(dc);
  HIPCHK(hipMemcpy(dc, code, words * 4, hipMemcpyHostToDevice));
  HIPCHK(hipMemset((uint32_t*)dc + words, 0, pad * 4));
  HIPCHK(hipMalloc(&di, nin * 2 + 2));
  c->vm_bufs.push_back(di);
  HIPCHK(hipMemcpy(di, in, nin * 2, hipMemcpyHostToDevice));
  HIPCHK(hipMalloc(&dout, nout * 2 + 2));
  c->vm_bufs.push_back(dout);
  HIPCHK(hipMemcpy(dout, out, nout * 2, hipMemcpyHostToDevice));
  d.code = (const uint4*)dc;
  d.nphases = nphases;
  d.in = (const uint16_t*)di;
  d.out = (const uint16_t*)dout;
  d.trace = nullptr;
  d.clk = nullptr;
  d.side = nullptr;
  if (side) {
    void* ds = nullptr;
    HIPCHK(hipMalloc(&ds, ((size_t)nphases + vm::PREFETCH) * W * 4));
    c->vm_bufs.push_back(ds);
    HIPCHK(hipMemcpy(ds, side, (size_t)nphases * W * 4, hipMemcpyHostToDevice));
    HIPCHK(hipMemset((uint32_t*)ds + (size_t)nphases * W, 0, (size_t)vm::PREFETCH * W * 4));
    d.side = (const uint32_t*)ds;
// ... 2847 lines not shown
```

Measured before the change: 1.779 million verifications/s.

## Compile inverse-free VM interpreters and add single-step rotated dispatch loop

Adds an INV template flag to the field-VM exec/run so programs statically asserted to have no inversion op get an interpreter with the fp_inv path compiled out. This is meant to cut code size and register pressure in the hot vote, fold and MSM kernels. It also adds a 1-step loop with a one-phase prefetch as the default for most runs, while the pool vote kernel keeps the 3-way unroll. vote_quad now takes TABLE as a runtime bool instead of instantiating two templates, which shrinks code but adds runtime selects.

```diff
diff --git a/consensus_overlord_amd/csrc/fpvm.hpp b/consensus_overlord_amd/csrc/fpvm.hpp
--- a/consensus_overlord_amd/csrc/fpvm.hpp
+++ b/consensus_overlord_amd/csrc/fpvm.hpp
@@ -275,6 +275,7 @@
 VM_FN uint32_t sign_mask(uint32_t w, int bit) { return (uint32_t)((int32_t)(w << (31 - bit)) >> 31); }
 VM_FN int coef5(uint32_t w, int lo) { return ((int)(w << (27 - lo))) >> 27; }
 
+template <bool INV = true>
 VM_FN void exec(const uint4 in, bool active, uint32_t* __restrict__ slots, const uint32_t* __restrict__ cst,
                 uint64_t scalar, const Out& out) {
   const uint32_t hdr = uniform(in.x);
@@ -339,12 +340,10 @@
       z = A.v[0] ? C : B;
     } else if (op >= OP_AND && op <= OP_XOR) {
       set_flag(z, op == OP_AND ? (A.v[0] & C.v[0]) : op == OP_OR ? (A.v[0] | C.v[0]) : (A.v[0] ^ C.v[0]));
-    } else if (op == OP_INV) {
-#ifndef OVH_VM_NO_INV
+    } else if (INV && op == OP_INV) {
       Fp a;
       canon(a, A);
       fp_inv(z, a, C);
-#endif
     }
     if (rare && op != OP_ST) st_slot(slots, dst, z);
   }
@@ -367,19 +366,26 @@
   }
 }
 
-template <bool SIDE = false>
+#ifndef OVH_VM_UNROLL
+#define OVH_VM_UNROLL 1
+#endif
+
+template <bool SIDE = false, bool INV = true, int UNROLL = OVH_VM_UNROLL>
 __device__ __forceinline__ void run(const uint4* __restrict__ code, uint32_t nphases, uint32_t W, uint32_t lane,
                                     bool active, uint32_t* __restrict__ slots, const uint32_t* __restrict__ cst,
                                     uint64_t scalar, const Out& out, uint64_t* __restrict__ trace = nullptr,
                                     const uint32_t* __restrict__ side = nullptr, uint32_t* __restrict__ scr = nullptr) {
   static_assert(PREFETCH >= 5, "the unrolled loops below read up to 4 phases past the end");
+  static_assert(UNROLL == 1 || UNROLL == 3, "loop shapes: 1 (rotated by moves) or 3 (unrolled over the rings)");
   if constexpr (SIDE) {
-    uint4 qa = code[lane], qb = code[W + lane], qc;
+    uint4 qa = code[lane], qb, qc;
     uint32_t sa = side[lane], sb = side[W + lane], sc;
+    if constexpr (UNROLL == 3) qb = code[W + lane];
     if (!active) sa = sb = 0;
     __builtin_amdgcn_s_waitcnt(0x0F70);
     auto step = [&](const uint4& q, uint4& q2, const uint32_t s, const uint32_t sn, uint32_t& s2,
                     const uint32_t ph) __attribute__((always_inline)) {
+      constexpr uint32_t QD = UNROLL == 3 ? 2 : 1;
       const bool fill = (sn & (SIDE_VALID | SIDE_FILL)) == (SIDE_VALID | SIDE_FILL);
       u32x4 f0, f1, f2;
       if (fill) {
@@ -388,9 +394,9 @@
         f1 = __builtin_nontemporal_load(src + 1);
         f2 = __builtin_nontemporal_load(src + 2);
       }
-      q2 = code[(size_t)(ph + 2) * W + lane];
+      q2 = code[(size_t)(ph + QD) * W + lane];
       s2 = active ? side[(size_t)(ph + 2) * W + lane] : 0u;
-      exec(q, active, slots, cst, scalar, out);
+      exec<INV>(q, active, slots, cst, scalar, out);
       side_spill(s, slots, scr);
       if (fill) {
         u32x4* d = reinterpret_cast<u32x4*>(slots + (sn & 0x7FF) * 12);
@@ -399,31 +405,50 @@
         d[2] = f2;
       }
     };
+    if constexpr (UNROLL == 3) {
 #pragma unroll 1
-    for (uint32_t ph = 0; ph < nphases; ph += 3) {
-      step(qa, qc, sa, sb, sc, ph);
-      step(qb, qa, sb, sc, sa, ph + 1);
-      step(qc, qb, sc, sa, sb, ph + 2);
+      for (uint32_t ph = 0; ph < nphases; ph += 3) {
+        step(qa, qc, sa, sb, sc, ph);
+        step(qb, qa, sb, sc, sa, ph + 1);
+        step(qc, qb, sc, sa, sb, ph + 2);
+      }
+    } else {
+#pragma unroll 1
+      for (uint32_t ph = 0; ph < nphases; ++ph) {
+        step(qa, qb, sa, sb, sc, ph);
+        qa = qb;
+        sa = sb;
+        sb = sc;
+      }
     }
     __asm__ volatile("s_waitcnt lgkmcnt(0)\n\ts_barrier" ::: "memory");
     return;
   }
   if (trace && threadIdx.x == 0) trace[0] = wall_clock64();
-  uint4 qa = code[lane], qb = code[W + lane], qc;
+  uint4 qa = code[lane], qb, qc;
+  if constexpr (UNROLL == 3) qb = code[W + lane];
   __builtin_amdgcn_s_waitcnt(0x0F70);
   auto step = [&](const uint4& q, uint4& q2, const uint32_t ph) __attribute__((always_inline)) {
-    q2 = code[(size_t)(ph + 2) * W + lane];
-    exec(q, active, slots, cst, scalar, out);
+    q2 = code[(size_t)(ph + (UNROLL == 3 ? 2 : 1)) * W + lane];
+    exec<INV>(q, active, slots, cst, scalar, out);
     if (trace && ph < nphases) {
       __asm__ volatile("s_waitcnt lgkmcnt(0)" ::: "memory");
       if (threadIdx.x == 0) trace[ph + 1] = wall_clock64();
     }
   };
+  if constexpr (UNROLL == 3) {
 #pragma unroll 1
-  for (uint32_t ph = 0; ph < nphases; ph += 3) {
-    step(qa, qc, ph);
-    step(qb, qa, ph + 1);
-    step(qc, qb, ph + 2);
+    for (uint32_t ph = 0; ph < nphases; ph += 3) {
+      step(qa, qc, ph);
+      step(qb, qa, ph + 1);
+      step(qc, qb, ph + 2);
+    }
+  } else {
+#pragma unroll 1
+    for (uint32_t ph = 0; ph < nphases; ++ph) {
+      step(qa, qb, ph);
+      qa = qb;
+    }
   }
   __asm__ volatile("s_waitcnt lgkmcnt(0)\n\ts_barrier" ::: "memory");
 }
diff --git a/consensus_overlord_amd/csrc/msm.hpp b/consensus_overlord_amd/csrc/msm.hpp
--- a/consensus_overlord_amd/csrc/msm.hpp
+++ b/consensus_overlord_amd/csrc/msm.hpp
@@ -169,7 +169,7 @@
     }
   }
   __syncthreads();
-  vm::run(prog.code, prog.nphases, W, lane, active, slots, cst, 0, vm::Out{nullptr, 0, 0});
+  vm::run<false, false>(prog.code, prog.nphases, W, lane, active, slots, cst, 0, vm::Out{nullptr, 0, 0});
   if (active) {
     const Slab& d = kd == SRC_U ? a.U : a.A;
     for (uint32_t k = lane; k < 6; k += W) {
diff --git a/consensus_overlord_amd/csrc/ovhip.hip b/consensus_overlord_amd/csrc/ovhip.hip
--- a/consensus_overlord_amd/csrc/ovhip.hip
+++ b/consensus_overlord_amd/csrc/ovhip.hip
@@ -27,6 +27,13 @@
 #include <vm_progs.inc>
 #endif
 static_assert(VM_KZERO == ovh::vm::KZERO && VM_KTAB == ovh::vm::KTAB, "fixed constants (tools/fpvm/gen.py)");
+#define VM_ASSERT_NO_INV(P) static_assert(!VM_##P##_HAS_INV, #P " has an inv op: it needs vm::run<SIDE, true>")
+#define VM_ASSERT_INV(P) static_assert(VM_##P##_HAS_INV, #P " has no inv op: bind it to vm::run<SIDE, false>")
+VM_ASSERT_NO_INV(MADD); VM_ASSERT_NO_INV(PADD); VM_ASSERT_NO_INV(G1PADD);
+VM_ASSERT_NO_INV(HDBL1); VM_ASSERT_NO_INV(HDBL2); VM_ASSERT_NO_INV(HDBL4); VM_ASSERT_NO_INV(HDBL8); VM_ASSERT_NO_INV(HDBL16);
+VM_ASSERT_NO_INV(VOTE1); VM_ASSERT_NO_INV(VOTE_T1); VM_ASSERT_NO_INV(VOTE1H); VM_ASSERT_NO_INV(VOTE_T1H);
+VM_ASSERT_NO_INV(VOTEW); VM_ASSERT_NO_INV(VOTEW_T);
+VM_ASSERT_NO_INV(VSAME); VM_ASSERT_NO_INV(VSAME_T); VM_ASSERT_NO_INV(VSAME8); VM_ASSERT_NO_INV(VSAME8_T);
 
 using namespace ovh;
 
@@ -234,6 +241,7 @@
 
 __device__ __forceinline__ uint32_t slot_flag_get(const uint32_t* slots, uint32_t s) { return slots[s * 12]; }
 
+template <int UNROLL = OVH_VM_UNROLL>
 __device__ __forceinline__ void fold_unit(uint32_t t, uint32_t m, const VmDev& prog, const uint32_t* cst,
                                           uint32_t* slots, uint32_t lane, bool active, Slab inF, Slab inS,
                                           Slab out, const int32_t* __restrict__ codes) {
@@ -253,7 +261,9 @@
     }
   }
   __syncthreads();
-  vm::run(prog.code, VM_FOLD_NPHASES, VM_FOLD_W, lane, active, slots, cst, 0, vm::Out{nullptr, 0, 0});
+  VM_ASSERT_NO_INV(FOLD);
+  vm::run<false, false, UNROLL>(prog.code, VM_FOLD_NPHASES, VM_FOLD_W, lane, active, slots, cst, 0,
+                                vm::Out{nullptr, 0, 0});
   if (active) {
     for (uint32_t k = lane; k < PART_PLANES; k += VM_FOLD_W) {
       Fp v;
@@ -528,11 +538,16 @@
   return reinterpret_cast<T*>(uni64(reinterpret_cast<uint64_t>(p)));
 }
 
-template <bool TABLE>
-__device__ __forceinline__ void vote_quad(const PoolArgs& a, uint32_t slot_in, uint32_t quad_in, uint32_t* lds) {
-  constexpr uint32_t NSLOTS = TABLE ? VM_VOTE_T_NSLOTS : VM_VOTE_NSLOTS;
-  constexpr uint32_t STRIDE = TABLE ? VOTE_T_STRIDE_W : VOTE_STRIDE_W;
-  constexpr uint32_t NPH = TABLE ? VM_VOTE_T_NPHASES : VM_VOTE_NPHASES;
+#ifndef OVH_POOL_UNROLL
+#define OVH_POOL_UNROLL 3
+#endif
+__device__ __forceinline__ void vote_quad(const PoolArgs& a, uint32_t slot_in, uint32_t quad_in, uint32_t* lds,
+                                          const bool TABLE) {
+  VM_ASSERT_NO_INV(VOTE);
+  VM_ASSERT_NO_INV(VOTE_T);
+  const uint32_t NSLOTS = TABLE ? VM_VOTE_T_NSLOTS : VM_VOTE_NSLOTS;
+  const uint32_t STRIDE = TABLE ? VOTE_T_STRIDE_W : VOTE_STRIDE_W;
+  const uint32_t NPH = TABLE ? VM_VOTE_T_NPHASES : VM_VOTE_NPHASES;
   const uint16_t* IN = TABLE ? VM_VOTE_T_IN : VM_VOTE_IN;
   const uint16_t* OUT = TABLE ? VM_VOTE_T_OUT : VM_VOTE_OUT;
   uint32_t* cst = lds;
@@ -573,7 +588,7 @@
     }
     __syncthreads();
     if (active) {
-      if constexpr (TABLE) {
+      if (TABLE) {
         const int32_t* idx = reinterpret_cast<const int32_t*>(sigs + (size_t)n * 144);
         const uint32_t e = uni(dget(&bd->has_idx)) ? (uint32_t)idx[i] : i;
         if (lane == 1) {
@@ -604,9 +619,10 @@
     }
     __syncthreads();
     const uint64_t scalar = vote_scalar(uni64(dget(&bd->seed)), uni64(dget(&bd->base)), i);
-    vm::run<true>(TABLE ? a.pt_code : a.pv_code, NPH, VM_VOTE_W, lane, active, slots, cst, scalar,
-                  vm::Out{s.p, s.cap, i}, nullptr, TABLE ? a.pt_side : a.pv_side,
-                  a.scr + (size_t)blockIdx.x * VM_SLICES * VOTE_NSCR * 12 + slice * VOTE_NSCR * 12);
+    vm::run<true, false, OVH_POOL_UNROLL>(
+        TABLE ? a.pt_code : a.pv_code, NPH, VM_VOTE_W, lane, active, slots, cst, scalar, vm::Out{s.p, s.cap, i},
+        nullptr, TABLE ? a.pt_side : a.pv_side,
+        a.scr + (size_t)blockIdx.x * VM_SLICES * VOTE_NSCR * 12 + slice * VOTE_NSCR * 12);
   }
   const uint32_t slot = uni(park[0]), quad = uni(park[1]) & 0x0FFFFFFFu, how = uni(park[1]) >> 28;
   const PoolBatch* bd = a.descs + slot;
@@ -627,7 +643,7 @@
     const uint32_t sg_grp = slot_flag_get(slots, OUT[TABLE ? VM_VOTE_T_OUT_SIG_GRP : VM_VOTE_OUT_SIG_GRP]);
     const uint32_t h_inf = slot_flag_get(slots, OUT[TABLE ? VM_VOTE_T_OUT_H_INF : VM_VOTE_OUT_H_INF]);
     uint32_t pk_parse, pk_inf, pk_grp;
-    if constexpr (TABLE) {
+    if (TABLE) {
       pk_parse = pf & PKF_PARSE;
       pk_inf = pf & PKF_INF;
       pk_grp = !(pf & PKF_GRP);
@@ -660,7 +676,7 @@
   const Slab s{unip(dgetp(&bd->state)), uni(dget(&bd->cap))};
   VmDev fold{};
   fold.code = a.fold_code;
-  fold_unit(quad, n, fold, cst, lds + SLOT_BASE_W, threadIdx.x % VM_FOLD_W, threadIdx.x < VM_FOLD_W,
+  fold_unit<1>(quad, n, fold, cst, lds + SLOT_BASE_W, threadIdx.x % VM_FOLD_W, threadIdx.x < VM_FOLD_W,
             Slab{s.p + (size_t)S_F * 12 * s.cap, s.cap}, Slab{nullptr, 0},
             Slab{unip(dgetp(&bd->part0)), uni(dget(&bd->part_cap))}, codes);
   if (pl) {
@@ -692,8 +708,7 @@
     slot = uni(slot);
     quad = uni(quad) | uni(how) << 28;
     __builtin_amdgcn_fence(__ATOMIC_ACQUIRE, "agent");
-    if (uni(dget(&a.descs[slot].table))) vote_quad<true>(a, slot, quad, lds);
-    else vote_quad<false>(a, slot, quad, lds);
+    vote_quad(a, slot, quad, lds, uni(dget(&a.descs[slot].table)) != 0);
   }
   if (a.wlog && threadIdx.x == 0 && blockIdx.x < PLOG_WGS) {
     uint64_t* w = a.wlog + (size_t)blockIdx.x * PLOG_WG_WORDS;
@@ -773,8 +788,9 @@
     slot_put(slots, VM_FINAL_IN[k], v.v);
   }
   __syncthreads();
-  vm::run(prog.code, VM_FINAL_NPHASES, VM_FINAL_W, lane, true, slots, cst, 0, vm::Out{nullptr, 0, 0},
-          blockIdx.x == 0 ? prog.trace : nullptr);
+  VM_ASSERT_INV(FINAL);
+  vm::run<false, true, 3>(prog.code, VM_FINAL_NPHASES, VM_FINAL_W, lane, true, slots, cst, 0, vm::Out{nullptr, 0, 0},
+                          blockIdx.x == 0 ? prog.trace : nullptr);
   if (lane == 0) *result = slot_flag_get(slots, VM_FINAL_OUT[0]) ? 1 : 0;
 }
 
@@ -838,7 +854,7 @@
     if constexpr (TABLE) slot_put(slots, IN[VM_VOTE_T1_IN_PK_X + (lane - 6)], v.v);
   }
   __syncthreads();
-  vm::run(prog.code, nph, 64, lane, true, slots, cst, scalar, vm::Out{s.p, s.cap, i});
+  vm::run<false, false>(prog.code, nph, 64, lane, true, slots, cst, scalar, vm::Out{s.p, s.cap, i});
   if (lane == 0) {
     const uint32_t sf = hdr[0], pf = hdr[1];
     const uint32_t sg_bad = sf & 1, sg_inf = (sf >> 1) & 1, sg_xz = (sf >> 2) & 1;
@@ -988,7 +1004,8 @@
   __syncthreads();
   constexpr uint32_t NPH = W8 ? (TABLE ? VM_VSAME8_T_NPHASES : VM_VSAME8_NPHASES)
                               : (TABLE ? VM_VSAME_T_NPHASES : VM_VSAME_NPHASES);
-  vm::run(prog.code, NPH, W, lane, active, slots, cst, vote_scalar(seed, base, i), vm::Out{s.p, s.cap, i});
+  vm::run<false, false>(prog.code, NPH, W, lane, active, slots, cst, vote_scalar(seed, base, i),
+                        vm::Out{s.p, s.cap, i});
   if (active && lane == 0) {
     const uint32_t sf = hdr[0], pf = hdr[1];
     const uint32_t sg_bad = sf & 1, sg_inf = (sf >> 1) & 1, sg_xz = (sf >> 2) & 1;
@@ -1034,7 +1051,8 @@
     slot_put(slots, VM_H2G_IN[lane], u.v);
   }
   __syncthreads();
-  vm::run(prog.code, VM_H2G_NPHASES, 16, lane, active, slots, cst, 0, vm::Out{g.p, g.cap, q});
+  VM_ASSERT_NO_INV(H2G);
+  vm::run<false, false>(prog.code, VM_H2G_NPHASES, 16, lane, active, slots, cst, 0, vm::Out{g.p, g.cap, q});
   if (active && lane == 0) ghinf[q] = slot_flag_get(slots, VM_H2G_OUT[VM_H2G_OUT_H_INF]) ? 1u : 0u;
 }
 
@@ -1076,7 +1094,7 @@
     }
   }
   __syncthreads();
-  vm::run(prog.code, prog.nphases, W, lane, active, slots, cst, 0, vm::Out{nullptr, 0, 0});
+  vm::run<false, false>(prog.code, prog.nphases, W, lane, active, slots, cst, 0, vm::Out{nullptr, 0, 0});
   if (active) {
     for (uint32_t k = lane; k < 3; k += W) {
       Fp v;
@@ -1138,7 +1156,8 @@
     }
     return;
   }
-  vm::run(prog.code, VM_GMIL_NPHASES, 64, lane, true, slots, cst, 0, vm::Out{g.p, g.cap, oq});
+  VM_ASSERT_NO_INV(GMIL);
+  vm::run<false, false>(prog.code, VM_GMIL_NPHASES, 64, lane, true, slots, cst, 0, vm::Out{g.p, g.cap, oq});
 }
 
 template <bool TABLE>
@@ -1202,7 +1221,8 @@
     if (lane == 0) *verdict = 0;
     return;
   }
-  vm::run(prog.code, VM_GFIN_NPHASES, 64, lane, true, slots, cst, 0, vm::Out{nullptr, 0, 0});
+  VM_ASSERT_INV(GFIN);
+  vm::run<false, true>(prog.code, VM_GFIN_NPHASES, 64, lane, true, slots, cst, 0, vm::Out{nullptr, 0, 0});
   if (lane == 0) *verdict = slot_flag_get(slots, VM_GFIN_OUT[0]) ? 1 : 0;
 }
 
@@ -1228,7 +1248,8 @@
     slot_put(slots, VM_QCPRE_IN[VM_QCPRE_IN_U00 + (lane - 2)], u.v);
   }
   __syncthreads();
-  vm::run(prog.code, VM_QCPRE_NPHASES, VM_QCPRE_W, lane, true, slots, cst, 0, vm::Out{s.p, s.cap, 0});
+  VM_ASSERT_NO_INV(QCPRE);
+  vm::run<false, false>(prog.code, VM_QCPRE_NPHASES, VM_QCPRE_W, lane, true, slots, cst, 0, vm::Out{s.p, s.cap, 0});
   if (lane == 0)
     *flags = hdr[0] | slot_flag_get(slots, VM_QCPRE_OUT[VM_QCPRE_OUT_SIG_OK]) << 8 |
              slot_flag_get(slots, VM_QCPRE_OUT[VM_QCPRE_OUT_SIG_GRP]) << 9 |
@@ -1251,7 +1272,8 @@
     slot_put(slots, VM_QCMIL_IN[lane], v.v);
   }
   __syncthreads();
-  vm::run(prog.code, VM_QCMIL_NPHASES, VM_QCMIL_W, lane, true, slots, cst, 0, vm::Out{s.p, s.cap, 1});
+  VM_ASSERT_NO_INV(QCMIL);
+  vm::run<false, false>(prog.code, VM_QCMIL_NPHASES, VM_QCMIL_W, lane, true, slots, cst, 0, vm::Out{s.p, s.cap, 1});
   if (lane == 0) {
     const uint32_t sf = *flags, kf = pk.flags[0];
     const uint32_t sg_bad = sf & 1, sg_inf = (sf >> 1) & 1, sg_xz = (sf >> 2) & 1;
@@ -1283,7 +1305,8 @@
     slot_put(slots, VM_FINAL1_IN[lane], v.v);
   }
   __syncthreads();
-  vm::run(prog.code, VM_FINAL1_NPHASES, VM_FINAL1_W, lane, true, slots, cst, 0, vm::Out{nullptr, 0, 0});
+  VM_ASSERT_INV(FINAL1);
+  vm::run<false, true>(prog.code, VM_FINAL1_NPHASES, VM_FINAL1_W, lane, true, slots, cst, 0, vm::Out{nullptr, 0, 0});
   return slot_flag_get(slots, VM_FINAL1_OUT[0]) != 0;
 }
 
@@ -1337,7 +1360,8 @@
     slot_put(slots, VM_FINAL_IN[k], v.v);
   }
   __syncthreads();
-  vm::run(prog.code, VM_FINAL_NPHASES, VM_FINAL_W, lane, true, slots, cst, 0, vm::Out{nullptr, 0, 0});
+  VM_ASSERT_INV(FINAL);
+  vm::run<false, true>(prog.code, VM_FINAL_NPHASES, VM_FINAL_W, lane, true, slots, cst, 0, vm::Out{nullptr, 0, 0});
   return slot_flag_get(slots, VM_FINAL_OUT[0]) != 0;
 }
 
@@ -1382,8 +1406,9 @@
     slot_put(slots, VM_RS_IN[lane], v.v);
   }
   __syncthreads();
-  vm::run(prog.code, VM_RS_NPHASES, VM_RS_W, lane, active, slots, cst, vote_scalar(seed, base, i),
-          vm::Out{s.p, s.cap, i});
+  VM_ASSERT_NO_INV(RS);
+  vm::run<false, false>(prog.code, VM_RS_NPHASES, VM_RS_W, lane, active, slots, cst, vote_scalar(seed, base, i),
+                        vm::Out{s.p, s.cap, i});
 }
 
 #define GROUPCHECK_FAIL (0x100 | BLST_POINT_NOT_IN_GROUP)
@@ -1409,7 +1434,8 @@
     hdr[0] = bad | inf << 1 | xz << 2;
   }
   __syncthreads();
-  vm::run(prog.code, VM_SIGCHK_NPHASES, VM_SIGCHK_W, lane, active, slots, cst, 0, vm::Out{nullptr, 0, 0});
+  VM_ASSERT_NO_INV(SIGCHK);
+  vm::run<false, false>(prog.code, VM_SIGCHK_NPHASES, VM_SIGCHK_W, lane, active, slots, cst, 0, vm::Out{nullptr, 0, 0});
   __syncthreads();
   if (!active) return;
   const uint32_t pf = hdr[0];
@@ -1460,7 +1486,7 @@
     }
   }
   __syncthreads();
-  vm::run(prog.code, prog.nphases, W, lane, active, slots, cst, 0, vm::Out{nullptr, 0, 0});
+  vm::run<false, false>(prog.code, prog.nphases, W, lane, active, slots, cst, 0, vm::Out{nullptr, 0, 0});
   if (active) {
     for (uint32_t k = lane; k < 6; k += W) {
       Fp v;
@@ -1512,7 +1538,8 @@
   for (int r = 0; r < 4; ++r) {
     if (active && lane < 3) slot_put(slots, VM_PKGEN_IN[lane], acc + lane * 12);
     __syncthreads();
-    vm::run(prog.code, VM_PKGEN_NPHASES, W, lane, active, slots, cst, k[r], vm::Out{nullptr, 0, 0});
+    VM_ASSERT_NO_INV(PKGEN);
+    vm::run<false, false>(prog.code, VM_PKGEN_NPHASES, W, lane, active, slots, cst, k[r], vm::Out{nullptr, 0, 0});
     __syncthreads();
     if (active && lane < 3) {
       Fp t;
@@ -1622,7 +1649,10 @@
   uint64_t d[4] = {0, 0, 0, 0};
   if (active)
     for (int j = 0; j < 4; ++j) d[j] = dig[j];
-  vm::run(p0.code, VM_SIGNG0_NPHASES, W, lane, active, slots, cst, signg_scalar(d, 0), vm::Out{nullptr, 0, 0});
+  VM_ASSERT_NO_INV(SIGNG0);
+  VM_ASSERT_NO_INV(SIGNG1);
+  vm::run<false, false>(p0.code, VM_SIGNG0_NPHASES, W, lane, active, slots, cst, signg_scalar(d, 0),
+                        vm::Out{nullptr, 0, 0});
   __syncthreads();
   if (active)
     for (uint32_t q = lane; q < 96; q += W)
@@ -1632,7 +1662,8 @@
     if (active)
       for (uint32_t q = lane; q < 96; q += W) slot_put(slots, VM_SIGNG1_IN[q], hst + q * 12);
     __syncthreads();
-    vm::run(p1.code, VM_SIGNG1_NPHASES, W, lane, active, slots, cst, signg_scalar(d, r), vm::Out{nullptr, 0, 0});
+    vm::run<false, false>(p1.code, VM_SIGNG1_NPHASES, W, lane, active, slots, cst, signg_scalar(d, r),
+                          vm::Out{nullptr, 0, 0});
     __syncthreads();
     if (active && lane < 6)
       for (int l = 0; l < 12; ++l) hst[lane * 12 + l] = slots[VM_SIGNG1_OUT[lane] * 12 + l];
@@ -1694,7 +1725,8 @@
     hdr[0] = bad | inf << 1 | xz << 2;
   }
   __syncthreads();
-  vm::run(prog.code, VM_PKCHK_NPHASES, VM_PKCHK_W, lane, active, slots, cst, 0, vm::Out{nullptr, 0, 0});
+  VM_ASSERT_NO_INV(PKCHK);
+  vm::run<false, false>(prog.code, VM_PKCHK_NPHASES, VM_PKCHK_W, lane, active, slots, cst, 0, vm::Out{nullptr, 0, 0});
   __syncthreads();
   if (!active) return;
   const uint32_t pf = hdr[0];
@@ -1741,7 +1773,7 @@
     }
   }
   __syncthreads();
-  vm::run(prog.code, prog.nphases, W, lane, active, slots, cst, 0, vm::Out{nullptr, 0, 0});
+  vm::run<false, false>(prog.code, prog.nphases, W, lane, active, slots, cst, 0, vm::Out{nullptr, 0, 0});
   if (active) {
     for (uint32_t k = lane; k < 3; k += W) {
       Fp v;
@@ -1782,7 +1814,8 @@
     slot_put(slots, VM_G1GRP_IN[lane], v.v);
   }
   __syncthreads();
-  vm::run(prog.code, VM_G1GRP_NPHASES, VM_G1GRP_W, lane, active, slots, cst, 0, vm::Out{nullptr, 0, 0});
+  VM_ASSERT_NO_INV(G1GRP);
+  vm::run<false, false>(prog.code, VM_G1GRP_NPHASES, VM_G1GRP_W, lane, active, slots, cst, 0, vm::Out{nullptr, 0, 0});
   if (active && lane == 0 && !(flags[0] & PKF_INF) && !slot_flag_get(slots, VM_G1GRP_OUT[VM_G1GRP_OUT_PK_GRP]))
     flags[0] |= PKF_GRP;
 }
@@ -1976,7 +2009,8 @@
     hdr[0] = bad | inf << 1 | xz << 2;
   }
   __syncthreads();
-  vm::run(prog.code, VM_PKDEC_NPHASES, W, lane, active, slots, cst, 0, vm::Out{nullptr, 0, 0});
+  VM_ASSERT_NO_INV(PKDEC);
+  vm::run<false, false>(prog.code, VM_PKDEC_NPHASES, W, lane, active, slots, cst, 0, vm::Out{nullptr, 0, 0});
   if (active && lane == 0) {
     const uint32_t pf = hdr[0];
     int32_t c = BLST_SUCCESS;
```

Result: faster. 1.805 million verifications/s, median of 6 (+1.5%).
